# PathologyFoundation/plip

Hardware: NVIDIA H100
Metric: image-text pairs/sec (224x224, 77-tok) (higher is better)
Workload: dtype bf16

## Files before the change

### include/plip_b200.h

```cpp
#ifndef PLIP_B200_H_
#define PLIP_B200_H_

#include <stdint.h>

#ifdef __cplusplus
extern "C" {
#endif

#define PLIP_API __attribute__((visibility("default")))

#define PLIP_B200_ABI_VERSION 5

#define PLIP_IMAGE_SIZE 224
#define PLIP_EMBED_DIM 512
#define PLIP_TEXT_SEQ 77
#define PLIP_VOCAB 49408

typedef struct plip_engine plip_engine_t;

enum plip_pixel_format {
  PLIP_PIX_F32_NCHW = 0,
  PLIP_PIX_BF16_NCHW = 1,
  PLIP_PIX_U8_NHWC = 2
};

enum plip_id_dtype { PLIP_IDS_I32 = 0, PLIP_IDS_I64 = 1 };

enum plip_operand_format { PLIP_OPERAND_BF16 = 0, PLIP_OPERAND_FP16 = 1 };

PLIP_API const char* plip_last_error(void);
PLIP_API int plip_abi_version(void);
PLIP_API uint64_t plip_launch_count(void);

typedef struct plip_tensor_info {
  char name[96];
  uint64_t offset;
  uint64_t numel;
  int32_t dtype;
  int32_t rows;
  int32_t cols;
  int32_t fused;
} plip_tensor_info_t;

PLIP_API int plip_weights_num_tensors(void);
PLIP_API int plip_weights_tensor_info(int index, plip_tensor_info_t* info);
PLIP_API uint64_t plip_weights_blob_bytes(void);

PLIP_API int plip_create(const void* host_blob, uint64_t blob_bytes, float logit_scale_exp, int device,
                         int max_micro_batch, plip_engine_t** out);
PLIP_API int plip_create_ex(const void* host_blob, uint64_t blob_bytes, float logit_scale_exp, int device,
                            int max_micro_batch, int operand_format, plip_engine_t** out);
PLIP_API int plip_destroy(plip_engine_t* e);
PLIP_API uint64_t plip_workspace_bytes(int max_micro_batch);
PLIP_API float plip_logit_scale_exp(const plip_engine_t* e);
PLIP_API int plip_max_micro_batch(const plip_engine_t* e);
PLIP_API int plip_operand_format(const plip_engine_t* e);
PLIP_API int plip_set_text_pooling(plip_engine_t* e, int no_eos_argmax);
PLIP_API int plip_set_last_layer_pruning(plip_engine_t* e, int on);
PLIP_API int plip_last_layer_pruning(const plip_engine_t* e);

PLIP_API int plip_encode_images(plip_engine_t* e, const void* pixels_dev, int pixel_format, int64_t n,
                                float* out_dev, int normalize, void* stream);

PLIP_API int plip_encode_images_hw(plip_engine_t* e, const void* pixels_dev, int pixel_format, int64_t n, int height,
                                   int width, float* out_dev, int normalize, void* stream);

PLIP_API int plip_encode_windows(plip_engine_t* e, const void* region_dev, int height, int width,
                                 int64_t row_pitch_bytes, const int32_t* origins_host, int64_t n, float* out_dev,
                                 int normalize, void* stream);
PLIP_API int plip_window_background_counts(const void* region_dev, int height, int width, int64_t row_pitch_bytes,
                                           const int32_t* origins_host, int64_t n, int threshold, int32_t* counts_dev,
                                           void* stream);
PLIP_API int plip_window_mask_counts(const void* mask_dev, int height, int width, int channels,
                                     int64_t row_pitch_bytes, const int32_t* origins_host, int64_t n, int threshold,
                                     int32_t* counts_dev, void* stream);

PLIP_API int plip_encode_text(plip_engine_t* e, const void* ids_dev, int ids_dtype,
                              const void* attention_mask_dev, int64_t n, int seq_len, float* out_dev,
                              int normalize, void* stream);

PLIP_API int plip_encode_text_prefix(plip_engine_t* e, const void* ids_dev, int ids_dtype,
                                     const void* attention_mask_dev, int64_t n, int seq_len, int prefix_len,
                                     float* out_dev, int normalize, void* stream);

typedef struct plip_tower_outputs {
  float* embeds;
  float* pooled;
  float* last_hidden;
  float* hidden;
  float* attn;
  int32_t normalize;
} plip_tower_outputs_t;
PLIP_API int plip_vision_outputs(plip_engine_t* e, const void* pixels_dev, int pixel_format, int64_t n, int height,
                                 int width, const plip_tower_outputs_t* outputs, void* stream);
PLIP_API int plip_text_outputs(plip_engine_t* e, const void* ids_dev, int ids_dtype, const void* attention_mask_dev,
                               int64_t n, int seq_len, const plip_tower_outputs_t* outputs, void* stream);

PLIP_API int plip_similarity(const float* img_dev, int64_t n, const float* txt_dev, int64_t m, float scale,
                             int normalize_img, int normalize_txt, float* logits_dev, int64_t ld_logits,
                             void* stream);

PLIP_API int plip_similarity_topk(const float* query_dev, int64_t n, const float* space_dev, int64_t m,
                                  float scale, int normalize_query, int normalize_space, int k,
                                  int32_t* idx_dev, float* val_dev, void* stream);

PLIP_API int plip_l2_normalize(float* x_dev, int64_t n, int dim, void* stream);

typedef struct plip_resize_desc {
  int64_t offset;
  int32_t width, height;
  int32_t new_width, new_height;
  int32_t left, top;
} plip_resize_desc_t;
PLIP_API int plip_resize_crop_u8(const void* src_dev, uint64_t src_bytes, const plip_resize_desc_t* descs_host,
                                 int64_t n, void* tiles_dev, void* stream);
PLIP_API int plip_resize_crop_bilinear_u8(const void* src_dev, uint64_t src_bytes, const plip_resize_desc_t* descs_host,
                                          int64_t n, void* tiles_dev, void* stream);
PLIP_API int plip_resize_crop_fill_u8(const void* src_dev, uint64_t src_bytes, const plip_resize_desc_t* descs_host,
                                      int64_t n, void* tiles_dev, void* stream);

PLIP_API int plip_mask_value_sets_u8(const void* masks_dev, int64_t n, int height, int width, int channels,
                                     uint32_t* sets_dev, void* stream);

typedef struct plip_warp_desc {
  double affine[6];
  double perspective[8];
  int32_t flip;
  int32_t apply_perspective;
  int32_t fill;
  int32_t reserved;
} plip_warp_desc_t;
PLIP_API int plip_warp_tiles_u8(const void* src_dev, void* dst_dev, const plip_warp_desc_t* descs_host, int64_t n,
                                void* stream);

PLIP_API int plip_resize_region_workspace(int height, int width, int new_height, int new_width, int out_row0,
                                          int out_row1, uint64_t* bytes);
PLIP_API int plip_resize_region_u8(const void* src_dev, int64_t src_row_pitch, int src_row0, int src_rows, int height,
                                   int width, void* out_dev, int64_t out_row_pitch, int new_height, int new_width,
                                   int out_row0, int out_row1, void* workspace_dev, uint64_t workspace_bytes,
                                   void* stream);
PLIP_API int plip_resize_filter_bounds(int in_size, int out_size, int32_t* bounds_host);

typedef struct plip_sgd_problem {
  double alpha;
  double pos_weight;
  double neg_weight;
  int32_t pos_class;
  int32_t sigma_index;
} plip_sgd_problem_t;
PLIP_API int plip_sgd_shuffle_permutation(int64_t n, uint32_t seed, int32_t* sigma_host);
PLIP_API int plip_sgd_workspace_bytes(int64_t n, int n_sigma, int n_problems, uint64_t* bytes);
PLIP_API int plip_sgd_fit(const float* x_dev, int64_t n, int dim, const int32_t* class_host, int n_classes,
                          const plip_sgd_problem_t* problems_host, int n_problems, const int32_t* sigma_host,
                          int n_sigma, int max_iter, double tol, int n_iter_no_change, float* coef_dev,
                          double* intercept_dev, int32_t* n_iter_dev, int32_t* overflow_dev, void* workspace_dev,
                          uint64_t workspace_bytes, void* stream);
PLIP_API int plip_linear_decision(const float* x_dev, int64_t n, int dim, const float* coef_dev,
                                  const double* intercept_dev, int n_out, float* scores_dev, int32_t* pred_dev,
                                  void* stream);

typedef struct plip_densenet plip_densenet_t;
PLIP_API int plip_densenet_num_tensors(void);
PLIP_API int plip_densenet_tensor_info(int index, plip_tensor_info_t* info);
PLIP_API uint64_t plip_densenet_blob_bytes(void);
PLIP_API uint64_t plip_densenet_workspace_bytes(int max_micro_batch);
PLIP_API int plip_densenet_create(const void* host_blob, uint64_t blob_bytes, int device, int max_micro_batch,
                                  plip_densenet_t** out);
PLIP_API int plip_densenet_destroy(plip_densenet_t* e);
PLIP_API int plip_densenet_max_micro_batch(const plip_densenet_t* e);
PLIP_API int plip_densenet_encode(plip_densenet_t* e, const void* tiles_dev, int64_t n, float* out_dev, void* stream);

PLIP_API int plip_encode_images_host(plip_engine_t* e, const void* pixels_host, int pixel_format, int64_t n,
                                     float* out_host, int normalize);
PLIP_API int plip_encode_text_host(plip_engine_t* e, const void* ids_host, int ids_dtype,
                                   const void* attention_mask_host, int64_t n, int seq_len,
                                   float* out_host, int normalize);

typedef struct plip_kernel_time {
  char name[48];
  int32_t launches;
  float total_ms;
  double flops;
  double bytes;
} plip_kernel_time_t;
PLIP_API int plip_profile_enable(plip_engine_t* e, int on);
PLIP_API int plip_profile_read(plip_engine_t* e, plip_kernel_time_t* out, int cap, int* count);

PLIP_API int plip_dbg_set_operand_format(int operand_format);
PLIP_API int plip_dbg_gemm(const void* A_bf16, int lda, const void* W_bf16, int ldw, int M, int N, int K,
                           const float* bias, void* out, int ldo, const float* pos, int epilogue, int cluster_size,
                           int block_n, const float* colsum, const float* stats_in, int n_partials, void* xb_out,
                           float* stats_out, void* stream);
PLIP_API int plip_dbg_resize_filter(int in_size, int out_size, int xx, int32_t* k_host, int k_cap, int* xmin,
                                    int* count);
PLIP_API int plip_dbg_resize_filter_bilinear(int in_size, int out_size, int xx, int32_t* k_host, int k_cap, int* xmin,
                                             int* count);
PLIP_API int plip_dbg_text_bucket_plan(const int32_t* lens_host, int64_t n, int seq_len, int32_t* perm_host,
                                       int32_t* bucket_start_host, int32_t* bucket_prefix_host, int cap);
PLIP_API int plip_dbg_rowstats_cast(const float* x, int64_t rows, int dim, void* xb_bf16, float* stats, void* stream);
PLIP_API int plip_dbg_layernorm(const float* x, int64_t rows, int dim, int64_t in_row_stride,
                                const float* gamma, const float* beta, float* out_f32, void* out_bf16,
                                void* stream);
PLIP_API int plip_dbg_attention(const void* qkv_bf16, int64_t n_seq, int seq_len, int heads, int causal,
                                const int32_t* key_mask, void* out_bf16, void* stream);
PLIP_API int plip_dbg_attention_probs(const void* qkv_bf16, int64_t n_seq, int seq_len, int heads, int causal,
                                      const int32_t* key_mask, float* probs_dev, void* stream);
PLIP_API int plip_dbg_densenet_op(int op, const void* in_dev, int lda, int64_t n, int side, int c_in, const void* w_dev,
                                  const float* a_scale, const float* a_shift, const float* e_scale,
                                  const float* e_shift, void* out_dev, int ldo, void* stream);
PLIP_API int plip_dbg_im2col(const void* pixels, int pixel_format, int64_t n, void* out_bf16, void* stream);
PLIP_API int plip_dbg_pos_interp(const float* pos_dev, int grid_h, int grid_w, float* out_dev, void* stream);
PLIP_API int plip_dbg_hidden_states_hw(plip_engine_t* e, const void* pixels_dev, int pixel_format, int64_t n,
                                       int height, int width, int num_layers, float* hidden_dev, void* stream);
PLIP_API int plip_dbg_hidden_states(plip_engine_t* e, int tower, const void* input_dev, int input_format,
                                    const void* attention_mask_dev, int64_t n, int num_layers,
                                    float* hidden_dev, void* stream);

#ifdef __cplusplus
}
#endif
#endif
```

### plip_b200/_lib.py

```python
from __future__ import annotations

import ctypes as C
from pathlib import Path

_PKG = Path(__file__).resolve().parent
LIB_PATH = _PKG / "libplip_b200.so"

_vp = C.c_void_p
_i = C.c_int
_i64 = C.c_int64
_u64 = C.c_uint64
_f = C.c_float
_fp = C.c_void_p


class TensorInfo(C.Structure):

    _fields_ = [
        ("name", C.c_char * 96),
        ("offset", C.c_uint64),
        ("numel", C.c_uint64),
        ("dtype", C.c_int32),
        ("rows", C.c_int32),
        ("cols", C.c_int32),
        ("fused", C.c_int32),
    ]


class KernelTime(C.Structure):

    _fields_ = [("name", C.c_char * 48), ("launches", C.c_int32), ("total_ms", C.c_float), ("flops", C.c_double),
                ("bytes", C.c_double)]


class ResizeDesc(C.Structure):

    _fields_ = [
        ("offset", C.c_int64),
        ("width", C.c_int32),
        ("height", C.c_int32),
        ("new_width", C.c_int32),
        ("new_height", C.c_int32),
        ("left", C.c_int32),
        ("top", C.c_int32),
    ]


class WarpDesc(C.Structure):

    _fields_ = [("affine", C.c_double * 6), ("perspective", C.c_double * 8), ("flip", C.c_int32),
                ("apply_perspective", C.c_int32), ("fill", C.c_int32), ("reserved", C.c_int32)]


class SgdProblem(C.Structure):

    _fields_ = [("alpha", C.c_double), ("pos_weight", C.c_double), ("neg_weight", C.c_double), ("pos_class", C.c_int32),
                ("sigma_index", C.c_int32)]


class TowerOutputs(C.Structure):

    _fields_ = [("embeds", C.c_void_p), ("pooled", C.c_void_p), ("last_hidden", C.c_void_p), ("hidden", C.c_void_p),
                ("attn", C.c_void_p), ("normalize", C.c_int32)]


SIGNATURES = {
    "plip_last_error": (C.c_char_p, []),
    "plip_abi_version": (_i, []),
    "plip_launch_count": (_u64, []),
    "plip_weights_num_tensors": (_i, []),
    "plip_weights_tensor_info": (_i, [_i, C.POINTER(TensorInfo)]),
    "plip_weights_blob_bytes": (_u64, []),
    "plip_create": (_i, [_vp, _u64, _f, _i, _i, C.POINTER(_vp)]),
    "plip_create_ex": (_i, [_vp, _u64, _f, _i, _i, _i, C.POINTER(_vp)]),
    "plip_operand_format": (_i, [_vp]),
    "plip_set_text_pooling": (_i, [_vp, _i]),
    "plip_set_last_layer_pruning": (_i, [_vp, _i]),
    "plip_last_layer_pruning": (_i, [_vp]),
    "plip_dbg_set_operand_format": (_i, [_i]),
    "plip_destroy": (_i, [_vp]),
    "plip_workspace_bytes": (_u64, [_i]),
    "plip_logit_scale_exp": (_f, [_vp]),
    "plip_max_micro_batch": (_i, [_vp]),
    "plip_encode_images": (_i, [_vp, _vp, _i, _i64, _fp, _i, _vp]),
    "plip_encode_images_hw": (_i, [_vp, _vp, _i, _i64, _i, _i, _fp, _i, _vp]),
    "plip_encode_windows": (_i, [_vp, _vp, _i, _i, _i64, _vp, _i64, _fp, _i, _vp]),
    "plip_window_background_counts": (_i, [_vp, _i, _i, _i64, _vp, _i64, _i, _vp, _vp]),
    "plip_encode_text": (_i, [_vp, _vp, _i, _vp, _i64, _i, _fp, _i, _vp]),
    "plip_encode_text_prefix": (_i, [_vp, _vp, _i, _vp, _i64, _i, _i, _fp, _i, _vp]),
    "plip_vision_outputs": (_i, [_vp, _vp, _i, _i64, _i, _i, C.POINTER(TowerOutputs), _vp]),
    "plip_text_outputs": (_i, [_vp, _vp, _i, _vp, _i64, _i, C.POINTER(TowerOutputs), _vp]),
    "plip_similarity": (_i, [_fp, _i64, _fp, _i64, _f, _i, _i, _fp, _i64, _vp]),
    "plip_similarity_topk": (_i, [_fp, _i64, _fp, _i64, _f, _i, _i, _i, _vp, _fp, _vp]),
    "plip_l2_normalize": (_i, [_fp, _i64, _i, _vp]),
    "plip_window_mask_counts": (_i, [_vp, _i, _i, _i, _i64, _vp, _i64, _i, _vp, _vp]),
    "plip_resize_crop_u8": (_i, [_vp, _u64, _vp, _i64, _vp, _vp]),
    "plip_resize_crop_bilinear_u8": (_i, [_vp, _u64, _vp, _i64, _vp, _vp]),
    "plip_resize_crop_fill_u8": (_i, [_vp, _u64, _vp, _i64, _vp, _vp]),
    "plip_mask_value_sets_u8": (_i, [_vp, _i64, _i, _i, _i, _vp, _vp]),
    "plip_warp_tiles_u8": (_i, [_vp, _vp, _vp, _i64, _vp]),
    "plip_resize_region_workspace": (_i, [_i, _i, _i, _i, _i, _i, C.POINTER(_u64)]),
    "plip_resize_region_u8": (_i, [_vp, _i64, _i, _i, _i, _i, _vp, _i64, _i, _i, _i, _i, _vp, _u64, _vp]),
    "plip_resize_filter_bounds": (_i, [_i, _i, _vp]),
    "plip_sgd_shuffle_permutation": (_i, [_i64, C.c_uint32, _vp]),
    "plip_sgd_workspace_bytes": (_i, [_i64, _i, _i, C.POINTER(_u64)]),
    "plip_sgd_fit": (_i, [_fp, _i64, _i, _vp, _i, _vp, _i, _vp, _i, _i, C.c_double, _i, _fp, _vp, _vp, _vp, _vp, _u64,
                          _vp]),
    "plip_linear_decision": (_i, [_fp, _i64, _i, _fp, _vp, _i, _fp, _vp, _vp]),
    "plip_densenet_num_tensors": (_i, []),
    "plip_densenet_tensor_info": (_i, [_i, C.POINTER(TensorInfo)]),
    "plip_densenet_blob_bytes": (_u64, []),
    "plip_densenet_workspace_bytes": (_u64, [_i]),
    "plip_densenet_create": (_i, [_vp, _u64, _i, _i, C.POINTER(_vp)]),
    "plip_densenet_destroy": (_i, [_vp]),
    "plip_densenet_max_micro_batch": (_i, [_vp]),
    "plip_densenet_encode": (_i, [_vp, _vp, _i64, _fp, _vp]),
    "plip_encode_images_host": (_i, [_vp, _vp, _i, _i64, _fp, _i]),
    "plip_encode_text_host": (_i, [_vp, _vp, _i, _vp, _i64, _i, _fp, _i]),
    "plip_profile_enable": (_i, [_vp, _i]),
    "plip_profile_read": (_i, [_vp, C.POINTER(KernelTime), _i, C.POINTER(_i)]),
    "plip_dbg_gemm": (_i, [_vp, _i, _vp, _i, _i, _i, _i, _fp, _vp, _i, _fp, _i, _i, _i, _fp, _fp, _i, _vp, _fp, _vp]),
    "plip_dbg_resize_filter": (_i, [_i, _i, _i, _vp, _i, C.POINTER(_i), C.POINTER(_i)]),
    "plip_dbg_resize_filter_bilinear": (_i, [_i, _i, _i, _vp, _i, C.POINTER(_i), C.POINTER(_i)]),
    "plip_dbg_text_bucket_plan": (_i, [_vp, _i64, _i, _vp, _vp, _vp, _i]),
    "plip_dbg_rowstats_cast": (_i, [_fp, _i64, _i, _vp, _fp, _vp]),
    "plip_dbg_layernorm": (_i, [_fp, _i64, _i, _i64, _fp, _fp, _fp, _vp, _vp]),
    "plip_dbg_attention": (_i, [_vp, _i64, _i, _i, _i, _vp, _vp, _vp]),
    "plip_dbg_attention_probs": (_i, [_vp, _i64, _i, _i, _i, _vp, _fp, _vp]),
    "plip_dbg_densenet_op": (_i, [_i, _vp, _i, _i64, _i, _i, _vp, _fp, _fp, _fp, _fp, _vp, _i, _vp]),
    "plip_dbg_im2col": (_i, [_vp, _i, _i64, _vp, _vp]),
    "plip_dbg_hidden_states": (_i, [_vp, _i, _vp, _i, _vp, _i64, _i, _fp, _vp]),
    "plip_dbg_pos_interp": (_i, [_fp, _i, _i, _fp, _vp]),
    "plip_dbg_hidden_states_hw": (_i, [_vp, _vp, _i, _i64, _i, _i, _i, _fp, _vp]),
}

_LIB = None


def lib(strict: bool = True) -> C.CDLL:
    global _LIB
    if _LIB is not None:
        return _LIB
    if not LIB_PATH.exists():
        raise RuntimeError(
            f"{LIB_PATH} is missing: build it with `python -m plip_b200.build` "
            "(plip_b200 has no CPU fallback; the sm_90a CUDA library is the product)."
        )
    dll = C.CDLL(str(LIB_PATH))
    missing = []
    for name, (res, args) in SIGNATURES.items():
        try:
            fn = getattr(dll, name)
        except AttributeError:
            missing.append(name)
            continue
        fn.restype = res
        fn.argtypes = args
    if missing and strict:
        raise RuntimeError(f"{LIB_PATH} does not export: {missing}")
    _LIB = dll
    return dll


def last_error() -> str:
    msg = lib(strict=False).plip_last_error()
    return msg.decode("utf-8", "replace") if msg else ""


def check(rc: int, what: str) -> None:
    if rc != 0:
        raise RuntimeError(f"{what} failed (rc={rc}): {last_error()}")
```

### plip_b200/csrc/engine.cu

```cuda
#include "kernels.cuh"

#include <stdlib.h>
#include <string.h>

#include <array>
#include <map>
#include <string>
#include <tuple>
#include <vector>

namespace plip {
const char* get_last_error();

namespace {

struct Spec {
  std::string name;
  int dtype;
  int rows, cols, fused;
  uint64_t offset, numel;
};

void add(std::vector<Spec>& v, const std::string& name, int dtype, int rows, int cols, int fused = 0) {
  Spec s;
  s.name = name; s.dtype = dtype; s.rows = rows; s.cols = cols; s.fused = fused;
  s.numel = (uint64_t)rows * cols;
  s.offset = 0;
  v.push_back(s);
}

void add_tower(std::vector<Spec>& v, const std::string& pfx, int D, int FF) {
  for (int l = 0; l < kLayers; ++l) {
    const std::string p = pfx + ".encoder.layers." + std::to_string(l);
    add(v, p + ".self_attn.q_proj.weight", 1, 3 * D, D, 3);
    add(v, p + ".self_attn.q_proj.bias", 0, 3 * D, 1, 3);
    add(v, p + ".self_attn.q_proj.colsum", 0, 3 * D, 1, 3);
    add(v, p + ".self_attn.out_proj.weight", 1, D, D);
    add(v, p + ".self_attn.out_proj.bias", 0, D, 1);
    add(v, p + ".mlp.fc1.weight", 1, FF, D, 2);
    add(v, p + ".mlp.fc1.bias", 0, FF, 1, 2);
    add(v, p + ".mlp.fc1.colsum", 0, FF, 1, 2);
    add(v, p + ".mlp.fc2.weight", 1, D, FF);
    add(v, p + ".mlp.fc2.bias", 0, D, 1);
  }
}

std::vector<Spec> build_specs() {
  std::vector<Spec> v;
  add(v, "vision_model.embeddings.patch_embedding.weight", 1, kVisDim, kPatchK);
  add(v, "vision_model.embeddings.class_embedding", 0, kVisDim, 1);
  add(v, "vision_model.embeddings.position_embedding.weight", 0, kVisSeq, kVisDim);
  add(v, "vision_model.pre_layrnorm.weight", 0, kVisDim, 1);
  add(v, "vision_model.pre_layrnorm.bias", 0, kVisDim, 1);
  add_tower(v, "vision_model", kVisDim, kVisFF);
  add(v, "vision_model.post_layernorm.weight", 0, kVisDim, 1);
  add(v, "vision_model.post_layernorm.bias", 0, kVisDim, 1);
  add(v, "visual_projection.weight", 1, kProj, kVisDim);
  add(v, "text_model.embeddings.token_embedding.weight", 0, kVocab, kTxtDim);
  add(v, "text_model.embeddings.position_embedding.weight", 0, kTxtSeq, kTxtDim);
  add_tower(v, "text_model", kTxtDim, kTxtFF);
  add(v, "text_model.final_layer_norm.weight", 0, kTxtDim, 1);
  add(v, "text_model.final_layer_norm.bias", 0, kTxtDim, 1);
  add(v, "text_projection.weight", 1, kProj, kTxtDim);
  uint64_t off = 0;
  for (auto& s : v) {
    s.offset = off;
    off += s.numel * (s.dtype == 1 ? 2 : 4);
    off = (off + 255) & ~255ull;
  }
  return v;
}

const std::vector<Spec>& specs() {
  static const std::vector<Spec> v = build_specs();
  return v;
}

uint64_t blob_bytes() {
  const auto& v = specs();
  const Spec& s = v.back();
  return (s.offset + s.numel * (s.dtype == 1 ? 2 : 4) + 255) & ~255ull;
}

struct LayerW {
  const float *bqkv, *sqkv, *bo, *b1, *s1, *b2;
  const __nv_bfloat16 *wqkv, *wo, *w1, *w2;
};

constexpr int kEosId = 49407;

enum ProfKind { PK_QKV = 0, PK_ATTN, PK_OUT, PK_FC1, PK_FC2, PK_PATCH, PK_IM2COL, PK_LN, PK_ROWSTATS, PK_EMBED, PK_PROJ,
                PK_MISC, PK_ATTN_LONG, PK_ATTN_PROBS, PK_COUNT };
const char* const kProfNames[PK_COUNT] = {"gemm[ln1+qkv]", "attention", "gemm[out_proj+resid]", "gemm[ln2+fc1+gelu]",
                                          "gemm[fc2+resid]", "gemm[patch_embed]", "im2col", "layernorm",
                                          "rowstats_cast", "text_embed", "gemm[projection]", "misc", "attention[long]",
                                          "attention[probs]"};

size_t pixel_bytes(int fmt, int height = kImage, int width = kImage) {
  const size_t px = (size_t)3 * height * width;
  return fmt == PLIP_PIX_F32_NCHW ? px * 4 : (fmt == PLIP_PIX_BF16_NCHW ? px * 2 : px);
}

struct VisGeom {
  int H = kImage, W = kImage, gh = kGrid, gw = kGrid, S = kVisSeq;
};

VisGeom vis_geom(int height, int width) {
  VisGeom g;
  g.H = height; g.W = width; g.gh = height / kPatch; g.gw = width / kPatch; g.S = g.gh * g.gw + 1;
  return g;
}

struct VisInput {
  const void* pixels;
  int fmt;
  WindowSrc win;
};

VisInput tiles(const void* pixels, int fmt) { return VisInput{pixels, fmt, WindowSrc{nullptr, 0, nullptr}}; }

int64_t images_per_pass(int max_mb, int S) {
  const int64_t n = (int64_t)kVisSeq * max_mb / S;
  return n < max_mb ? n : max_mb;
}

struct GraphKey {
  int tower;
  int n;
  int format;
  int normalize, seq_len, prefix_len, has_mask, pool_argmax, prune;
  auto fields() const {
    return std::tie(tower, n, format, normalize, seq_len, prefix_len, has_mask, pool_argmax, prune);
  }
  bool operator<(const GraphKey& o) const { return fields() < o.fields(); }
};

struct Graph {
  cudaGraphExec_t exec = nullptr;
  unsigned long long kernels = 0;
};

}
}

using namespace plip;

struct plip_engine {
  int device = 0;
  int max_mb = 0;
  int text_pool_argmax = 0;
  int prune_last = 0;
  int f16 = 0;
  float logit_scale_exp = 1.f;
  uint8_t* d_blob = nullptr;
  const __nv_bfloat16 *v_patch_w = nullptr, *v_proj = nullptr;
  const float *v_cls = nullptr, *v_pos = nullptr, *v_pre_g = nullptr, *v_pre_b = nullptr, *v_post_g = nullptr,
              *v_post_b = nullptr;
  LayerW vis[kLayers], txt[kLayers];
  const float *t_tok = nullptr, *t_pos = nullptr, *t_fin_g = nullptr, *t_fin_b = nullptr;
  const __nv_bfloat16* t_proj = nullptr;
  float* X = nullptr;
  __nv_bfloat16* Xn = nullptr;
  __nv_bfloat16* AO = nullptr;
  float2* stats = nullptr;
  __nv_bfloat16* QKV = nullptr;
  __nv_bfloat16* H = nullptr;
  __nv_bfloat16* pooled = nullptr;
  int32_t* row_idx = nullptr;
  int32_t* kmask = nullptr;
  cudaEvent_t ev_last = nullptr;
  cudaStream_t s_compute = nullptr, s_copy = nullptr;
  cudaEvent_t ev_copied[2] = {nullptr, nullptr}, ev_done[2] = {nullptr, nullptr};
  void* d_in[2] = {nullptr, nullptr};
  size_t d_in_bytes = 0;
  void* h_stage[2] = {nullptr, nullptr};
  size_t h_stage_bytes = 0;
  float* d_out = nullptr;
  size_t d_out_bytes = 0;
  void* d_aux = nullptr;
  size_t d_aux_bytes = 0;
  int32_t* d_win = nullptr;
  size_t d_win_bytes = 0;
  int graph_max_n = 128;
  cudaStream_t s_cap = nullptr;
  void* g_in[2] = {nullptr, nullptr};
  size_t g_in_bytes[2] = {0, 0};
  float* g_out = nullptr;
  std::map<GraphKey, Graph> graphs;
  bool prof_on = false;
  int prof_tower = 0;
  std::vector<cudaEvent_t> prof_ev;
  struct ProfRec { int kind; int tower; double flops, bytes; };
  std::vector<ProfRec> prof_rec;
};

namespace {

struct ProfScope {
  plip_engine* e;
  cudaStream_t st;
  bool on;
  ProfScope(plip_engine* e_, cudaStream_t st_, int kind, double flops, double bytes) : e(e_), st(st_), on(e_->prof_on) {
    if (!on) return;
    if (e->prof_rec.size() >= 8192) { on = false; return; }
    cudaEvent_t a = nullptr, b = nullptr;
    if (cudaEventCreate(&a) != cudaSuccess || cudaEventCreate(&b) != cudaSuccess) { on = false; return; }
    e->prof_ev.push_back(a);
    e->prof_ev.push_back(b);
    e->prof_rec.push_back({kind, e->prof_tower, flops, bytes});
    cudaEventRecord(a, st);
  }
  ~ProfScope() {
    if (on) cudaEventRecord(e->prof_ev.back(), st);
  }
};

template <typename T>
const T* wptr(const plip_engine* e, const Spec& s) {
  return reinterpret_cast<const T*>(e->d_blob + s.offset);
}

int bind_weights(plip_engine* e) {
  const auto& v = specs();
  size_t i = 0;
  auto nextf = [&]() { return wptr<float>(e, v[i++]); };
  auto nextb = [&]() { return wptr<__nv_bfloat16>(e, v[i++]); };
  auto tower = [&](LayerW* L) {
    for (int l = 0; l < kLayers; ++l) {
      L[l].wqkv = nextb(); L[l].bqkv = nextf(); L[l].sqkv = nextf();
      L[l].wo = nextb(); L[l].bo = nextf();
      L[l].w1 = nextb(); L[l].b1 = nextf(); L[l].s1 = nextf();
      L[l].w2 = nextb(); L[l].b2 = nextf();
    }
  };
  e->v_patch_w = nextb();
  e->v_cls = nextf();
  e->v_pos = nextf();
  e->v_pre_g = nextf(); e->v_pre_b = nextf();
  tower(e->vis);
  e->v_post_g = nextf(); e->v_post_b = nextf();
  e->v_proj = nextb();
  e->t_tok = nextf();
  e->t_pos = nextf();
  tower(e->txt);
  e->t_fin_g = nextf(); e->t_fin_b = nextf();
  e->t_proj = nextb();
  PLIP_REQUIRE(i == v.size(), "internal: weight table mismatch (%zu vs %zu)", i, v.size());
  return 0;
}

struct WsLayout {
  size_t x, xn, ao, stats, qkv, h, pooled, rowidx, kmask, total;
};

WsLayout ws_layout(int mb) {
  const size_t rv = (size_t)mb * kVisSeq, rt = (size_t)mb * kTxtSeq;
  auto mx = [](size_t a, size_t b) { return a > b ? a : b; };
  auto al = [](size_t a) { return (a + 1023) & ~(size_t)1023; };
  WsLayout w;
  size_t off = 0;
  w.x = off; off += al(mx(rv * kVisDim, rt * kTxtDim) * 4);
  w.xn = off; off += al(mx(rv * kVisDim, rt * kTxtDim) * 2);
  w.ao = off; off += al(mx(rv * kVisDim, rt * kTxtDim) * 2);
  w.stats = off; off += al(mx(rv, rt) * kStatSlots * sizeof(float2));
  w.qkv = off; off += al(mx(rv * 3 * kVisDim, rt * 3 * kTxtDim) * 2);
  w.h = off; off += al(mx(mx(rv * kVisFF, rt * kTxtFF), (size_t)mb * kPatches * kPatchK) * 2);
  w.pooled = off; off += al((size_t)mb * kVisDim * 2);
  w.rowidx = off; off += al((size_t)mb * 4);
  w.kmask = off; off += al(rt * 4);
  w.total = off;
  return w;
}

int gemm(plip_engine* e, int kind, GemmArgs g, cudaStream_t st) {
  g.f16 = e->f16;
  const double M = g.M, N = g.N, K = g.K;
  const double out_elem = g.epi == EPI_BIAS_RESID_F32 ? 8 : (g.epi == EPI_F32 || g.epi == EPI_PATCH_F32 ? 4 : 2);
  ProfScope ps(e, st, kind, 2 * M * N * K, M * K * 2 + N * K * 2 + M * N * out_elem + (g.xb_out ? M * N * 2 : 0));
  return launch_gemm(g, st);
}

int layer_tail(plip_engine* e, const LayerW& w, int rows, int D, int FF, const __nv_bfloat16* ao, float* x, bool last,
               int& np, cudaStream_t st) {
  GemmArgs g;
  g.A = ao; g.lda = D; g.W = w.wo; g.ldw = D; g.M = rows; g.N = D; g.K = D;
  g.bias = w.bo; g.out = x; g.ldo = D; g.epi = EPI_BIAS_RESID_F32;
  g.xb_out = e->Xn; g.stats_out = e->stats; g.n_tiles_used = &np;
  if (int rc = gemm(e, PK_OUT, g, st)) return rc;
  g = GemmArgs();
  g.A = e->Xn; g.lda = D; g.W = w.w1; g.ldw = D; g.M = rows; g.N = FF; g.K = D;
  g.bias = w.b1; g.colsum = w.s1; g.stats_in = e->stats; g.n_partials = np;
  g.out = e->H; g.ldo = FF; g.epi = EPI_LN_BIAS_GELU_BF16;
  if (int rc = gemm(e, PK_FC1, g, st)) return rc;
  g = GemmArgs();
  g.A = e->H; g.lda = FF; g.W = w.w2; g.ldw = FF; g.M = rows; g.N = D; g.K = FF;
  g.bias = w.b2; g.out = x; g.ldo = D; g.epi = EPI_BIAS_RESID_F32;
  if (!last) { g.xb_out = e->Xn; g.stats_out = e->stats; g.n_tiles_used = &np; }
  return gemm(e, PK_FC2, g, st);
}

struct PassOut {
  float *embeds = nullptr, *pooled = nullptr, *last_hidden = nullptr;
  float* hidden = nullptr;
  int64_t hidden_stride = 0;
  float* attn = nullptr;
  int64_t attn_stride = 0;
  int normalize = 0;
};

PassOut pass_out(const plip_tower_outputs_t& o, int64_t n, int64_t i0, int S, int D, int heads) {
  PassOut p;
  const int64_t tok = (int64_t)S * D, pp = (int64_t)heads * S * S;
  if (o.embeds) p.embeds = o.embeds + i0 * kProj;
  if (o.pooled) p.pooled = o.pooled + i0 * D;
  if (o.last_hidden) p.last_hidden = o.last_hidden + i0 * tok;
  if (o.hidden) { p.hidden = o.hidden + i0 * tok; p.hidden_stride = n * tok; }
  if (o.attn) { p.attn = o.attn + i0 * pp; p.attn_stride = n * pp; }
  p.normalize = o.normalize;
  return p;
}

PassOut embeds_only(float* out, int normalize) {
  PassOut p;
  p.embeds = out;
  p.normalize = normalize;
  return p;
}

int run_layers(plip_engine* e, const LayerW* L, int64_t n_seq, int S, int D, int FF, int heads, bool causal,
               const int32_t* kmask, int num_layers, cudaStream_t st, bool prune = false,
               const int32_t* pool_idx = nullptr, const PassOut& out = PassOut(), const float** pooled_x = nullptr) {
  const int64_t M = n_seq * S;
  PLIP_REQUIRE(M <= 0x7fffffff / 4, "micro-batch too large");
  PLIP_REQUIRE(!prune || (pooled_x && !out.hidden && !out.attn), "internal: per-layer outputs of a pruned pass");
  const size_t x_bytes = (size_t)M * D * 4;
  if (out.hidden) PLIP_CUDA_CHECK(cudaMemcpyAsync(out.hidden, e->X, x_bytes, cudaMemcpyDeviceToDevice, st));
  if (num_layers <= 0) return 0;
  {
    ProfScope ps(e, st, PK_ROWSTATS, 0, (double)M * D * 6 + (double)M * 8);
    if (int rc = launch_rowstats_cast(e->X, M, D, e->Xn, e->stats, e->f16, st)) return rc;
  }
  const double b_att = (double)M * 3 * D * 2 + (double)M * D * 2;
  const double f_att = 4.0 * (double)n_seq * heads * S * S * kHeadDim;
  int np = 1;
  for (int l = 0; l < num_layers; ++l) {
    const LayerW& w = L[l];
    const bool last = l + 1 == num_layers;
    GemmArgs g;
    g.A = e->Xn; g.lda = D; g.W = w.wqkv; g.ldw = D; g.M = (int)M; g.N = 3 * D; g.K = D;
    g.bias = w.bqkv; g.colsum = w.sqkv; g.stats_in = e->stats; g.n_partials = np;
    g.out = e->QKV; g.ldo = 3 * D; g.epi = EPI_LN_BIAS_BF16;
    if (int rc = gemm(e, PK_QKV, g, st)) return rc;
    {
      ProfScope ps(e, st, S > 128 ? PK_ATTN_LONG : PK_ATTN, f_att, b_att);
      if (int rc = launch_attention(e->QKV, n_seq, S, heads, causal, kmask, e->AO, e->f16, st)) return rc;
    }
    if (out.attn) {
      ProfScope ps(e, st, PK_ATTN_PROBS, 0.5 * f_att, (double)M * 2 * D * 2 + (double)n_seq * heads * S * S * 4);
      if (int rc = launch_attention_probs(e->QKV, n_seq, S, heads, causal, kmask, out.attn + l * out.attn_stride,
                                          e->f16, st)) return rc;
    }
    if (!(prune && last)) {
      if (int rc = layer_tail(e, w, (int)M, D, FF, e->AO, e->X, last, np, st)) return rc;
      if (out.hidden)
        PLIP_CUDA_CHECK(cudaMemcpyAsync(out.hidden + (l + 1) * out.hidden_stride, e->X, x_bytes,
                                        cudaMemcpyDeviceToDevice, st));
      continue;
    }
    __nv_bfloat16* ao_p = e->QKV;
    float* x_p = reinterpret_cast<float*>(reinterpret_cast<uint8_t*>(e->QKV) + (((size_t)n_seq * D * 2 + 1023) & ~(size_t)1023));
    {
      ProfScope ps(e, st, PK_MISC, 0, (double)n_seq * D * 12);
      if (int rc = launch_gather_rows(e->AO, e->X, pool_idx, S, n_seq, D, ao_p, x_p, st)) return rc;
    }
    if (int rc = layer_tail(e, w, (int)n_seq, D, FF, ao_p, x_p, true, np, st)) return rc;
    *pooled_x = x_p;
  }
  return 0;
}

int vision_trunk(plip_engine* e, const VisInput& in, int64_t mb, const VisGeom& geo, int num_layers,
                 cudaStream_t st, bool prune = false, const PassOut& out = PassOut(),
                 const float** pooled_x = nullptr) {
  e->prof_tower = 0;
  const double dmb = (double)mb;
  const int patches = geo.gh * geo.gw;
  const float* pos = e->v_pos;
  if (geo.gh != kGrid || geo.gw != kGrid) {
    float* table = reinterpret_cast<float*>(e->QKV);
    ProfScope ps(e, st, PK_MISC, 0, (double)kVisSeq * kVisDim * 4 + (double)geo.S * kVisDim * 4);
    if (int rc = launch_pos_interp(e->v_pos, geo.gh, geo.gw, table, st)) return rc;
    pos = table;
  }
  {
    ProfScope ps(e, st, PK_IM2COL, 0, dmb * (double)pixel_bytes(in.fmt, geo.H, geo.W) + dmb * patches * kPatchK * 2);
    const int rc = in.win.region ? launch_window_im2col(in.win, mb, e->H, e->f16, st)
                                 : launch_im2col(in.pixels, in.fmt, mb, geo.H, geo.W, e->H, e->f16, st);
    if (rc) return rc;
  }
  GemmArgs g;
  g.A = e->H; g.lda = kPatchK; g.W = e->v_patch_w; g.ldw = kPatchK;
  g.M = (int)(mb * patches); g.N = kVisDim; g.K = kPatchK;
  g.out = e->X; g.ldo = kVisDim; g.pos = pos; g.patches = patches; g.seq = geo.S; g.epi = EPI_PATCH_F32;
  if (int rc = gemm(e, PK_PATCH, g, st)) return rc;
  {
    ProfScope ps(e, st, PK_MISC, 0, dmb * kVisDim * 4);
    if (int rc = launch_cls_rows(e->v_cls, pos, mb, geo.S, e->X, st)) return rc;
  }
  const int64_t M = mb * geo.S;
  {
    ProfScope ps(e, st, PK_LN, 0, (double)M * kVisDim * 8);
    if (int rc = launch_layernorm(e->X, nullptr, kVisDim, M, kVisDim, e->v_pre_g, e->v_pre_b, e->X, nullptr, e->f16, st)) return rc;
  }
  return run_layers(e, e->vis, mb, geo.S, kVisDim, kVisFF, kVisHeads, false, nullptr, num_layers, st, prune, nullptr,
                    out, pooled_x);
}

int pooled_head(plip_engine* e, const float* pooled_x, const int32_t* pool_idx, int64_t mb, int S, int D,
                const float* gamma, const float* beta, const __nv_bfloat16* proj, float* out, int normalize,
                cudaStream_t st, float* pooled_f32) {
  {
    ProfScope ps(e, st, PK_LN, 0, (double)mb * D * (pooled_f32 ? 10 : 6));
    const bool compact = pooled_x != nullptr;
    if (int rc = launch_layernorm(compact ? pooled_x : e->X, compact ? nullptr : pool_idx,
                                  compact || pool_idx ? (int64_t)D : (int64_t)S * D, mb, D, gamma, beta, pooled_f32,
                                  e->pooled, e->f16, st)) return rc;
  }
  if (!out) return 0;
  GemmArgs g;
  g.A = e->pooled; g.lda = D; g.W = proj; g.ldw = D;
  g.M = (int)mb; g.N = kProj; g.K = D; g.out = out; g.ldo = kProj; g.epi = EPI_F32;
  if (int rc = gemm(e, PK_PROJ, g, st)) return rc;
  if (normalize) {
    ProfScope ps(e, st, PK_MISC, 0, (double)mb * kProj * 8);
    return launch_l2_normalize(out, mb, kProj, st);
  }
  return 0;
}

int vision_pass(plip_engine* e, const VisInput& in, int64_t mb, const VisGeom& geo, const PassOut& out, bool prune,
                cudaStream_t st) {
  const float* pooled_x = nullptr;
  if (int rc = vision_trunk(e, in, mb, geo, kLayers, st, prune, out, &pooled_x)) return rc;
  if (out.last_hidden)
    PLIP_CUDA_CHECK(cudaMemcpyAsync(out.last_hidden, e->X, (size_t)mb * geo.S * kVisDim * 4, cudaMemcpyDeviceToDevice,
                                    st));
  if (!out.embeds && !out.pooled) return 0;
  return pooled_head(e, pooled_x, nullptr, mb, geo.S, kVisDim, e->v_post_g, e->v_post_b, e->v_proj, out.embeds,
                     out.normalize, st, out.pooled);
}

int text_trunk(plip_engine* e, const void* ids, int ids_dtype, const void* mask, int64_t mb, int S, int stride,
               int num_layers, cudaStream_t st, bool prune = false, const PassOut& out = PassOut(),
               const float** pooled_x = nullptr) {
  e->prof_tower = 1;
  {
    ProfScope ps(e, st, PK_EMBED, 0, (double)mb * S * kTxtDim * 8);
    if (int rc = launch_text_embed(ids, ids_dtype, mb, S, stride, e->t_tok, e->t_pos, e->X, e->row_idx, kEosId, e->text_pool_argmax, st)) return rc;
  }
  const int32_t* km = nullptr;
  if (mask) {
    ProfScope ps(e, st, PK_MISC, 0, (double)mb * S * 12);
    if (int rc = launch_mask_to_i32(mask, ids_dtype, mb * S, S, stride, e->kmask, st)) return rc;
    km = e->kmask;
  }
  return run_layers(e, e->txt, mb, S, kTxtDim, kTxtFF, kTxtHeads, true, km, num_layers, st, prune, e->row_idx, out,
                    pooled_x);
}

int text_pass(plip_engine* e, const void* ids, int ids_dtype, const void* mask, int64_t mb, int S, int stride,
              const PassOut& out, bool prune, cudaStream_t st) {
  const float* pooled_x = nullptr;
  if (int rc = text_trunk(e, ids, ids_dtype, mask, mb, S, stride, kLayers, st, prune, out, &pooled_x)) return rc;
  if (out.last_hidden) {
    ProfScope ps(e, st, PK_LN, 0, (double)mb * S * kTxtDim * 8);
    if (int rc = launch_layernorm(e->X, nullptr, kTxtDim, mb * S, kTxtDim, e->t_fin_g, e->t_fin_b, out.last_hidden,
                                  nullptr, e->f16, st)) return rc;
  }
  if (!out.embeds && !out.pooled) return 0;
  return pooled_head(e, pooled_x, e->row_idx, mb, S, kTxtDim, e->t_fin_g, e->t_fin_b, e->t_proj, out.embeds,
                     out.normalize, st, out.pooled);
}

int ensure_host_path(plip_engine* e) {
  if (e->s_compute) return 0;
  PLIP_CUDA_CHECK(cudaStreamCreateWithFlags(&e->s_compute, cudaStreamNonBlocking));
  PLIP_CUDA_CHECK(cudaStreamCreateWithFlags(&e->s_copy, cudaStreamNonBlocking));
  for (int i = 0; i < 2; ++i) {
    PLIP_CUDA_CHECK(cudaEventCreateWithFlags(&e->ev_copied[i], cudaEventDisableTiming));
    PLIP_CUDA_CHECK(cudaEventCreateWithFlags(&e->ev_done[i], cudaEventDisableTiming));
  }
  return 0;
}

int grow_dev(void** p, size_t* have, size_t want) {
  if (*have >= want) return 0;
  if (*p) PLIP_CUDA_CHECK(cudaFree(*p));
  *p = nullptr; *have = 0;
  PLIP_CUDA_CHECK(cudaMalloc(p, want));
  *have = want;
  return 0;
}

constexpr long long kMinBucketRows = 8192, kBucketOverheadRows = 2048;
constexpr int kMaxTextBuckets = 8;

int plan_text_buckets(const int32_t* lens, int64_t n, int seq_len, int32_t* perm, int32_t* start, int32_t* prefix,
                      int cap) {
  std::vector<int64_t> upto(seq_len + 1, 0);
  for (int64_t i = 0; i < n; ++i) {
    const int L = lens[i] < 1 ? 1 : (lens[i] > seq_len ? seq_len : lens[i]);
    ++upto[L];
  }
  std::vector<int64_t> first(seq_len + 2, 0);
  for (int L = 1; L <= seq_len; ++L) first[L + 1] = first[L] + upto[L];
  if (perm) {
    std::vector<int64_t> cur(first.begin(), first.end());
    for (int64_t i = 0; i < n; ++i) {
      const int L = lens[i] < 1 ? 1 : (lens[i] > seq_len ? seq_len : lens[i]);
      perm[cur[L]++] = (int32_t)i;
    }
  }
  std::vector<int> ends;
  for (int L = 1; L <= seq_len; ++L)
    if (upto[L]) ends.push_back(L);
  for (int L = 1; L <= seq_len; ++L) upto[L] += upto[L - 1];
  const int m = (int)ends.size();
  const int kb = cap < kMaxTextBuckets ? cap : kMaxTextBuckets;
  const long long INF = 1LL << 62;
  std::vector<std::vector<long long>> f(kb, std::vector<long long>(m, INF));
  std::vector<std::vector<int>> from(kb, std::vector<int>(m, -1));
  auto cost = [&](int jlo, int jhi) {
    const long long cnt = upto[ends[jhi]] - (jlo ? upto[ends[jlo - 1]] : 0);
    const long long rows = cnt * ends[jhi];
    return (rows < kMinBucketRows ? kMinBucketRows : rows) + kBucketOverheadRows;
  };
  for (int j = 0; j < m; ++j) f[0][j] = cost(0, j);
  for (int b = 1; b < kb; ++b)
    for (int j = b; j < m; ++j)
      for (int i = b - 1; i < j; ++i)
        if (f[b - 1][i] < INF) {
          const long long c = f[b - 1][i] + cost(i + 1, j);
          if (c < f[b][j]) f[b][j] = c, from[b][j] = i;
        }
  int best_b = 0;
  for (int b = 1; b < kb; ++b)
    if (m > b && f[b][m - 1] < f[best_b][m - 1]) best_b = b;
  const int nb = best_b + 1;
  int j = m - 1;
  for (int b = best_b; b >= 0; --b) {
    prefix[b] = ends[j];
    const int i = b ? from[b][j] : -1;
    start[b] = (int32_t)(i >= 0 ? upto[ends[i]] : 0);
    j = i;
  }
  start[nb] = (int32_t)n;
  return nb;
}

bool is_pinned(const void* p) {
  cudaPointerAttributes a;
  if (cudaPointerGetAttributes(&a, p) != cudaSuccess) {
    cudaGetLastError();
    return false;
  }
  return a.type == cudaMemoryTypeHost;
}

}

namespace {

int count_kernel_nodes(cudaGraph_t g, unsigned long long* kernels) {
  size_t n = 0;
  PLIP_CUDA_CHECK(cudaGraphGetNodes(g, nullptr, &n));
  std::vector<cudaGraphNode_t> nodes(n);
  PLIP_CUDA_CHECK(cudaGraphGetNodes(g, nodes.data(), &n));
  *kernels = 0;
  for (cudaGraphNode_t node : nodes) {
    cudaGraphNodeType type;
    PLIP_CUDA_CHECK(cudaGraphNodeGetType(node, &type));
    *kernels += type == cudaGraphNodeTypeKernel;
  }
  return 0;
}

template <typename F>
int capture_graph(plip_engine* e, F&& body, Graph* out) {
  if (!e->s_cap) PLIP_CUDA_CHECK(cudaStreamCreateWithFlags(&e->s_cap, cudaStreamNonBlocking));
  PLIP_CUDA_CHECK(cudaStreamBeginCapture(e->s_cap, cudaStreamCaptureModeThreadLocal));
  int rc = body(e->s_cap);
  cudaGraph_t g = nullptr;
  const cudaError_t ce = cudaStreamEndCapture(e->s_cap, &g);
  if (g) {
    const int rc_count = count_kernel_nodes(g, &out->kernels);
    if (rc == 0) rc = rc_count;
    g_launch_count.fetch_sub(out->kernels, std::memory_order_relaxed);
  }
  if (rc != 0) {
    if (g) cudaGraphDestroy(g);
    return rc;
  }
  PLIP_CUDA_CHECK(ce);
  const cudaError_t ci = cudaGraphInstantiate(&out->exec, g, 0);
  cudaGraphDestroy(g);
  PLIP_CUDA_CHECK(ci);
  return 0;
}

int check_pixels(const char* fn, const plip_engine* e, const void* in, const void* out, int fmt, int64_t n,
                 int height, int width) {
  PLIP_REQUIRE(in && out, "%s: null argument", fn);
  PLIP_REQUIRE(n > 0, "%s: n must be positive (got %lld)", fn, (long long)n);
  PLIP_REQUIRE(fmt >= 0 && fmt <= 2, "%s: unknown pixel format %d", fn, fmt);
  PLIP_REQUIRE(height >= kPatch && width >= kPatch && height / kPatch <= kMaxGrid && width / kPatch <= kMaxGrid,
               "%s: image size %dx%d out of range (32 <= height, width and at most %d patches of 32 per side)", fn,
               height, width, kMaxGrid);
  PLIP_REQUIRE(e != nullptr, "%s: null engine", fn);
  const int S = (height / kPatch) * (width / kPatch) + 1;
  PLIP_REQUIRE(S <= (int64_t)kVisSeq * e->max_mb,
               "%s: a %dx%d image has %d tokens, more than the %lld token rows of the workspace "
               "(%d x max_micro_batch %d); create the engine with max_micro_batch >= %d",
               fn, height, width, S, (long long)kVisSeq * e->max_mb, kVisSeq, e->max_mb, (S + kVisSeq - 1) / kVisSeq);
  return 0;
}

int check_ids(const char* fn, const plip_engine* e, const void* ids, const void* out, int ids_dtype, int64_t n,
              int seq_len, int prefix_len) {
  PLIP_REQUIRE(ids && out, "%s: null argument", fn);
  PLIP_REQUIRE(n > 0, "%s: n must be positive (got %lld)", fn, (long long)n);
  PLIP_REQUIRE(seq_len >= 1 && seq_len <= kTxtSeq,
               "Sequence length must be less than max_position_embeddings (got `sequence length`: %d and "
               "max_position_embeddings: %d)", seq_len, kTxtSeq);
  PLIP_REQUIRE(prefix_len >= 1 && prefix_len <= seq_len, "%s: prefix_len %d out of [1,%d]", fn, prefix_len, seq_len);
  PLIP_REQUIRE(ids_dtype == PLIP_IDS_I32 || ids_dtype == PLIP_IDS_I64, "%s: unknown ids dtype %d", fn, ids_dtype);
  PLIP_REQUIRE(e != nullptr, "%s: null engine", fn);
  return 0;
}

int check_outputs(const char* fn, const plip_tower_outputs_t* o) {
  PLIP_REQUIRE(o != nullptr, "%s: null outputs", fn);
  PLIP_REQUIRE(o->embeds || o->pooled || o->last_hidden || o->hidden || o->attn, "%s: no output requested", fn);
  return 0;
}

int check_windows(const char* fn, const void* region, int height, int width, int64_t row_pitch,
                  const int32_t* origins, int64_t n, const void* out, int channels = 3) {
  PLIP_REQUIRE(region && origins && out, "%s: null argument", fn);
  PLIP_REQUIRE(n > 0, "%s: n must be positive (got %lld)", fn, (long long)n);
  PLIP_REQUIRE(height >= kImage && width >= kImage, "%s: region %dx%d is smaller than one %dx%d window", fn, height,
               width, kImage, kImage);
  PLIP_REQUIRE(row_pitch >= (int64_t)channels * width, "%s: row pitch %lld bytes < %d * width = %lld", fn,
               (long long)row_pitch, channels, (long long)channels * width);
  for (int64_t i = 0; i < n; ++i) {
    const int r = origins[2 * i], c = origins[2 * i + 1];
    PLIP_REQUIRE(r >= 0 && c >= 0 && r <= height - kImage && c <= width - kImage,
                 "%s: window %lld at (%d, %d) is outside the %dx%d region (rows 0..%d, columns 0..%d)", fn,
                 (long long)i, r, c, height, width, height - kImage, width - kImage);
  }
  return 0;
}

template <typename F>
int micro_batches(plip_engine* e, int64_t n, int64_t per_pass, cudaStream_t st, F&& pass) {
  PLIP_CUDA_CHECK(cudaStreamWaitEvent(st, e->ev_last, 0));
  for (int64_t i = 0; i < n; i += per_pass)
    if (int rc = pass(i, n - i < per_pass ? n - i : per_pass)) return rc;
  PLIP_CUDA_CHECK(cudaEventRecord(e->ev_last, st));
  return 0;
}

bool graph_eligible(const plip_engine* e, int64_t n) {
  return e->graph_max_n > 0 && n <= e->graph_max_n && n <= e->max_mb && !e->prof_on;
}

constexpr size_t kMaxGraphs = 96;
void trim_graphs(plip_engine* e) {
  if (e->graphs.size() < kMaxGraphs) return;
  cudaDeviceSynchronize();
  for (auto& kv : e->graphs) cudaGraphExecDestroy(kv.second.exec);
  e->graphs.clear();
}

struct Staged {
  const void* src;
  size_t bytes;
};

template <typename F>
int graph_call(plip_engine* e, const GraphKey& key, std::array<Staged, 2> in, float* out, cudaStream_t st,
               F&& forward) {
  PLIP_CUDA_CHECK(cudaStreamWaitEvent(st, e->ev_last, 0));
  auto it = e->graphs.find(key);
  if (it == e->graphs.end()) {
    const size_t stage_bytes[2] = {(size_t)e->graph_max_n * pixel_bytes(PLIP_PIX_F32_NCHW),
                                   (size_t)e->graph_max_n * kTxtSeq * 8};
    for (int i = 0; i < 2; ++i)
      if (in[i].src)
        if (int rc = grow_dev(&e->g_in[i], &e->g_in_bytes[i], stage_bytes[i])) return rc;
    if (!e->g_out) PLIP_CUDA_CHECK(cudaMalloc(&e->g_out, (size_t)e->graph_max_n * kProj * 4));
    if (int rc = forward(st, in[0].src, in[1].src, out)) return rc;
    Graph graph;
    if (int rc = capture_graph(e, [&](cudaStream_t cs) {
          return forward(cs, in[0].src ? e->g_in[0] : nullptr, in[1].src ? e->g_in[1] : nullptr, e->g_out);
        }, &graph)) return rc;
    trim_graphs(e);
    e->graphs.emplace(key, graph);
  } else {
    for (int i = 0; i < 2; ++i)
      if (in[i].src) PLIP_CUDA_CHECK(cudaMemcpyAsync(e->g_in[i], in[i].src, in[i].bytes, cudaMemcpyDeviceToDevice, st));
    PLIP_CUDA_CHECK(cudaGraphLaunch(it->second.exec, st));
    PLIP_CUDA_CHECK(cudaMemcpyAsync(out, e->g_out, (size_t)key.n * kProj * 4, cudaMemcpyDeviceToDevice, st));
    g_launch_count.fetch_add(it->second.kernels, std::memory_order_relaxed);
  }
  PLIP_CUDA_CHECK(cudaEventRecord(e->ev_last, st));
  return 0;
}

int dbg_hidden_states(const char* fn, plip_engine* e, int tower, const void* in, int fmt, const void* mask, int64_t n,
                      int height, int width, int num_layers, float* hidden, cudaStream_t st) {
  PLIP_REQUIRE(tower == 0 || tower == 1, "%s: tower %d out of range (0 vision, 1 text)", fn, tower);
  PLIP_REQUIRE(num_layers >= 0 && num_layers <= kLayers, "%s: num_layers %d out of range", fn, num_layers);
  if (int rc = tower == 0 ? check_pixels(fn, e, in, hidden, fmt, n, height, width)
                          : check_ids(fn, e, in, hidden, fmt, n, kTxtSeq, kTxtSeq)) return rc;
  const VisGeom geo = vis_geom(height, width);
  const int S = tower == 0 ? geo.S : kTxtSeq, D = tower == 0 ? kVisDim : kTxtDim;
  const int64_t per_pass = tower == 0 ? images_per_pass(e->max_mb, S) : e->max_mb;
  PLIP_REQUIRE(n <= per_pass, "%s: n=%lld sequences of %d tokens exceed one pass (%lld)", fn, (long long)n, S,
               (long long)per_pass);
  return micro_batches(e, n, n, st, [&](int64_t, int64_t) {
    if (int rc = tower == 0 ? vision_trunk(e, tiles(in, fmt), n, geo, num_layers, st)
                            : text_trunk(e, in, fmt, mask, n, kTxtSeq, kTxtSeq, num_layers, st)) return rc;
    PLIP_CUDA_CHECK(cudaMemcpyAsync(hidden, e->X, (size_t)n * S * D * 4, cudaMemcpyDeviceToDevice, st));
    return 0;
  });
}

}

extern "C" {

PLIP_API const char* plip_last_error(void) { return plip::get_last_error(); }
PLIP_API int plip_abi_version(void) { return PLIP_B200_ABI_VERSION; }
PLIP_API uint64_t plip_launch_count(void) { return plip::g_launch_count.load(std::memory_order_relaxed); }

PLIP_API int plip_weights_num_tensors(void) { return (int)specs().size(); }

PLIP_API int plip_weights_tensor_info(int index, plip_tensor_info_t* info) {
  const auto& v = specs();
  PLIP_REQUIRE(info != nullptr && index >= 0 && index < (int)v.size(), "tensor_info: index %d out of range", index);
  memset(info, 0, sizeof(*info));
  strncpy(info->name, v[index].name.c_str(), sizeof(info->name) - 1);
  info->offset = v[index].offset;
  info->numel = v[index].numel;
  info->dtype = v[index].dtype;
  info->rows = v[index].rows;
  info->cols = v[index].cols;
  info->fused = v[index].fused;
  return 0;
}

PLIP_API uint64_t plip_weights_blob_bytes(void) { return blob_bytes(); }

PLIP_API uint64_t plip_workspace_bytes(int max_micro_batch) {
  return max_micro_batch > 0 ? ws_layout(max_micro_batch).total : 0;
}

PLIP_API int plip_create(const void* host_blob, uint64_t nbytes, float logit_scale_exp, int device,
                         int max_micro_batch, plip_engine_t** out) {
  return plip_create_ex(host_blob, nbytes, logit_scale_exp, device, max_micro_batch, PLIP_OPERAND_BF16, out);
}

PLIP_API int plip_create_ex(const void* host_blob, uint64_t nbytes, float logit_scale_exp, int device,
                            int max_micro_batch, int operand_format, plip_engine_t** out) {
  PLIP_REQUIRE(out != nullptr && host_blob != nullptr, "plip_create: null argument");
  PLIP_REQUIRE(operand_format == PLIP_OPERAND_BF16 || operand_format == PLIP_OPERAND_FP16,
               "plip_create: unknown operand format %d", operand_format);
  PLIP_REQUIRE(nbytes == blob_bytes(), "plip_create: blob is %llu bytes, expected %llu",
               (unsigned long long)nbytes, (unsigned long long)blob_bytes());
  PLIP_REQUIRE(max_micro_batch >= 1 && max_micro_batch <= 8192, "plip_create: max_micro_batch %d out of [1,8192]",
               max_micro_batch);
  int ndev = 0;
  PLIP_CUDA_CHECK(cudaGetDeviceCount(&ndev));
  PLIP_REQUIRE(device >= 0 && device < ndev, "plip_create: device %d not present (%d devices)", device, ndev);
  PLIP_CUDA_CHECK(cudaSetDevice(device));
  cudaDeviceProp prop;
  PLIP_CUDA_CHECK(cudaGetDeviceProperties(&prop, device));
  PLIP_REQUIRE(prop.major == 9 && prop.minor == 0, "plip_create: device %d is sm_%d%d; this library is built for sm_90a only",
               device, prop.major, prop.minor);
  plip_engine* e = new plip_engine();
  e->device = device;
  e->max_mb = max_micro_batch;
  e->f16 = operand_format == PLIP_OPERAND_FP16 ? 1 : 0;
  if (const char* gm = getenv("PLIP_GRAPH_MAX")) e->graph_max_n = atoi(gm) < 0 ? 0 : (atoi(gm) > 1024 ? 1024 : atoi(gm));
  e->logit_scale_exp = logit_scale_exp;
  const WsLayout w = ws_layout(max_micro_batch);
  uint8_t* ws = nullptr;
  cudaError_t ce = cudaEventCreateWithFlags(&e->ev_last, cudaEventDisableTiming);
  if (ce == cudaSuccess) ce = cudaMalloc(&e->d_blob, nbytes);
  if (ce == cudaSuccess) ce = cudaMalloc(&ws, w.total);
  e->X = reinterpret_cast<float*>(ws);
  if (ce != cudaSuccess) {
    set_last_error("plip_create: allocating %llu (weights) + %llu (workspace) bytes on device %d failed: %s",
                   (unsigned long long)nbytes, (unsigned long long)w.total, device, cudaGetErrorString(ce));
    cudaGetLastError();
    plip_destroy(e);
    return -1;
  }
  e->Xn = reinterpret_cast<__nv_bfloat16*>(ws + w.xn);
  e->AO = reinterpret_cast<__nv_bfloat16*>(ws + w.ao);
  e->stats = reinterpret_cast<float2*>(ws + w.stats);
  e->QKV = reinterpret_cast<__nv_bfloat16*>(ws + w.qkv);
  e->H = reinterpret_cast<__nv_bfloat16*>(ws + w.h);
  e->pooled = reinterpret_cast<__nv_bfloat16*>(ws + w.pooled);
  e->row_idx = reinterpret_cast<int32_t*>(ws + w.rowidx);
  e->kmask = reinterpret_cast<int32_t*>(ws + w.kmask);
  ce = cudaMemcpy(e->d_blob, host_blob, nbytes, cudaMemcpyHostToDevice);
  if (ce != cudaSuccess) {
    set_last_error("plip_create: weight upload failed: %s", cudaGetErrorString(ce));
    plip_destroy(e);
    return -1;
  }
  if (bind_weights(e) != 0) {
    plip_destroy(e);
    return -1;
  }
  *out = e;
  return 0;
}

PLIP_API int plip_destroy(plip_engine_t* e) {
  if (!e) return 0;
  cudaSetDevice(e->device);
  cudaDeviceSynchronize();
  if (e->d_blob) cudaFree(e->d_blob);
  if (e->X) cudaFree(e->X);
  for (int i = 0; i < 2; ++i) {
    if (e->d_in[i]) cudaFree(e->d_in[i]);
    if (e->h_stage[i]) cudaFreeHost(e->h_stage[i]);
    if (e->ev_copied[i]) cudaEventDestroy(e->ev_copied[i]);
    if (e->ev_done[i]) cudaEventDestroy(e->ev_done[i]);
  }
  if (e->d_out) cudaFree(e->d_out);
  if (e->d_aux) cudaFree(e->d_aux);
  if (e->d_win) cudaFree(e->d_win);
  if (e->ev_last) cudaEventDestroy(e->ev_last);
  for (auto& kv : e->graphs) cudaGraphExecDestroy(kv.second.exec);
  for (void* p : e->g_in)
    if (p) cudaFree(p);
  if (e->g_out) cudaFree(e->g_out);
  if (e->s_cap) cudaStreamDestroy(e->s_cap);
  for (cudaEvent_t ev : e->prof_ev) cudaEventDestroy(ev);
  if (e->s_compute) cudaStreamDestroy(e->s_compute);
  if (e->s_copy) cudaStreamDestroy(e->s_copy);
  delete e;
  return 0;
}

PLIP_API int plip_profile_enable(plip_engine_t* e, int on) {
  PLIP_REQUIRE(e != nullptr, "plip_profile_enable: null engine");
  for (cudaEvent_t ev : e->prof_ev) cudaEventDestroy(ev);
  e->prof_ev.clear();
  e->prof_rec.clear();
  e->prof_on = on != 0;
  return 0;
}

PLIP_API int plip_profile_read(plip_engine_t* e, plip_kernel_time_t* out, int cap, int* count) {
  PLIP_REQUIRE(e && out && count && cap > 0, "plip_profile_read: bad argument");
  plip_kernel_time_t agg[2 * PK_COUNT];
  memset(agg, 0, sizeof(agg));
  for (size_t i = 0; i < e->prof_rec.size(); ++i) {
    PLIP_CUDA_CHECK(cudaEventSynchronize(e->prof_ev[2 * i + 1]));
    float ms = 0.f;
    PLIP_CUDA_CHECK(cudaEventElapsedTime(&ms, e->prof_ev[2 * i], e->prof_ev[2 * i + 1]));
    plip_kernel_time_t& a = agg[e->prof_rec[i].tower * PK_COUNT + e->prof_rec[i].kind];
    a.launches += 1;
    a.total_ms += ms;
    a.flops += e->prof_rec[i].flops;
    a.bytes += e->prof_rec[i].bytes;
  }
  int n = 0;
  for (int t = 0; t < 2; ++t)
    for (int k = 0; k < PK_COUNT; ++k) {
      const plip_kernel_time_t& a = agg[t * PK_COUNT + k];
      if (a.launches == 0) continue;
      if (n < cap) {
        out[n] = a;
        snprintf(out[n].name, sizeof(out[n].name), "%s/%s", t == 0 ? "vision" : "text", kProfNames[k]);
      }
      ++n;
    }
  *count = n;
  return 0;
}

PLIP_API float plip_logit_scale_exp(const plip_engine_t* e) { return e ? e->logit_scale_exp : 0.f; }
PLIP_API int plip_max_micro_batch(const plip_engine_t* e) { return e ? e->max_mb : 0; }
PLIP_API int plip_operand_format(const plip_engine_t* e) { return e ? e->f16 : -1; }
PLIP_API int plip_set_text_pooling(plip_engine_t* e, int no_eos_argmax) {
  PLIP_REQUIRE(e != nullptr, "plip_set_text_pooling: null engine");
  e->text_pool_argmax = no_eos_argmax != 0;
  return 0;
}

PLIP_API int plip_set_last_layer_pruning(plip_engine_t* e, int on) {
  PLIP_REQUIRE(e != nullptr, "plip_set_last_layer_pruning: null engine");
  e->prune_last = on != 0;
  return 0;
}
PLIP_API int plip_last_layer_pruning(const plip_engine_t* e) { return e ? e->prune_last : -1; }

PLIP_API int plip_encode_images(plip_engine_t* e, const void* pixels_dev, int pixel_format, int64_t n,
                                float* out_dev, int normalize, void* stream) {
  return plip_encode_images_hw(e, pixels_dev, pixel_format, n, kImage, kImage, out_dev, normalize, stream);
}

PLIP_API int plip_encode_images_hw(plip_engine_t* e, const void* pixels_dev, int pixel_format, int64_t n, int height,
                                   int width, float* out_dev, int normalize, void* stream) {
  if (int rc = check_pixels("plip_encode_images_hw", e, pixels_dev, out_dev, pixel_format, n, height, width)) return rc;
  const VisGeom geo = vis_geom(height, width);
  const size_t pb = pixel_bytes(pixel_format, height, width);
  const bool prune = e->prune_last != 0;
  cudaStream_t st = static_cast<cudaStream_t>(stream);
  if (height == kImage && width == kImage && graph_eligible(e, n)) {
    const GraphKey key{0, (int)n, pixel_format, normalize ? 1 : 0, 0, 0, 0, 0, e->prune_last};
    return graph_call(e, key, {{{pixels_dev, (size_t)n * pb}, {nullptr, 0}}}, out_dev, st,
                      [&](cudaStream_t s, const void* pixels, const void*, float* out) {
                        return vision_pass(e, tiles(pixels, pixel_format), n, geo, embeds_only(out, normalize), prune,
                                           s);
                      });
  }
  return micro_batches(e, n, images_per_pass(e->max_mb, geo.S), st, [&](int64_t i, int64_t mb) {
    return vision_pass(e, tiles(static_cast<const uint8_t*>(pixels_dev) + i * pb, pixel_format), mb, geo,
                       embeds_only(out_dev + i * kProj, normalize), prune, st);
  });
}

PLIP_API int plip_encode_windows(plip_engine_t* e, const void* region_dev, int height, int width,
                                 int64_t row_pitch_bytes, const int32_t* origins_host, int64_t n, float* out_dev,
                                 int normalize, void* stream) {
  if (int rc = check_windows("plip_encode_windows", region_dev, height, width, row_pitch_bytes, origins_host, n,
                             out_dev)) return rc;
  PLIP_REQUIRE(e != nullptr, "plip_encode_windows: null engine");
  cudaStream_t st = static_cast<cudaStream_t>(stream);
  PLIP_CUDA_CHECK(cudaStreamWaitEvent(st, e->ev_last, 0));
  if (int rc = grow_dev(reinterpret_cast<void**>(&e->d_win), &e->d_win_bytes, (size_t)n * 2 * sizeof(int32_t)))
    return rc;
  PLIP_CUDA_CHECK(cudaMemcpyAsync(e->d_win, origins_host, (size_t)n * 2 * sizeof(int32_t), cudaMemcpyHostToDevice, st));
  const bool prune = e->prune_last != 0;
  const uint8_t* region = static_cast<const uint8_t*>(region_dev);
  return micro_batches(e, n, images_per_pass(e->max_mb, kVisSeq), st, [&](int64_t i, int64_t mb) {
    const VisInput in{nullptr, PLIP_PIX_U8_NHWC, WindowSrc{region, row_pitch_bytes, e->d_win + 2 * i}};
    return vision_pass(e, in, mb, VisGeom(), embeds_only(out_dev + i * kProj, normalize), prune, st);
  });
}

PLIP_API int plip_window_background_counts(const void* region_dev, int height, int width, int64_t row_pitch_bytes,
                                           const int32_t* origins_host, int64_t n, int threshold, int32_t* counts_dev,
                                           void* stream) {
  if (int rc = check_windows("plip_window_background_counts", region_dev, height, width, row_pitch_bytes,
                             origins_host, n, counts_dev)) return rc;
  return launch_window_background(static_cast<const uint8_t*>(region_dev), row_pitch_bytes, origins_host, n, threshold,
                                  counts_dev, static_cast<cudaStream_t>(stream));
}

PLIP_API int plip_window_mask_counts(const void* mask_dev, int height, int width, int channels,
                                     int64_t row_pitch_bytes, const int32_t* origins_host, int64_t n, int threshold,
                                     int32_t* counts_dev, void* stream) {
  PLIP_REQUIRE(channels == 1 || channels == 3, "plip_window_mask_counts: channels must be 1 or 3 (got %d)", channels);
  if (int rc = check_windows("plip_window_mask_counts", mask_dev, height, width, row_pitch_bytes, origins_host, n,
                             counts_dev, channels)) return rc;
  return launch_window_mask(static_cast<const uint8_t*>(mask_dev), row_pitch_bytes, channels, origins_host, n,
                            threshold, counts_dev, static_cast<cudaStream_t>(stream));
}

PLIP_API int plip_encode_text(plip_engine_t* e, const void* ids_dev, int ids_dtype, const void* attention_mask_dev,
                              int64_t n, int seq_len, float* out_dev, int normalize, void* stream) {
  return plip_encode_text_prefix(e, ids_dev, ids_dtype, attention_mask_dev, n, seq_len, seq_len, out_dev, normalize,
                                 stream);
}

PLIP_API int plip_encode_text_prefix(plip_engine_t* e, const void* ids_dev, int ids_dtype,
                                     const void* attention_mask_dev, int64_t n, int seq_len, int prefix_len,
                                     float* out_dev, int normalize, void* stream) {
  if (int rc = check_ids("plip_encode_text", e, ids_dev, out_dev, ids_dtype, n, seq_len, prefix_len)) return rc;
  const size_t row = (size_t)seq_len * (ids_dtype == PLIP_IDS_I64 ? 8 : 4);
  const bool prune = e->prune_last != 0;
  cudaStream_t st = static_cast<cudaStream_t>(stream);
  if (graph_eligible(e, n)) {
    const GraphKey key{1, (int)n, ids_dtype, normalize ? 1 : 0, seq_len, prefix_len, attention_mask_dev ? 1 : 0,
                       e->text_pool_argmax, e->prune_last};
    return graph_call(e, key, {{{ids_dev, n * row}, {attention_mask_dev, n * row}}}, out_dev, st,
                      [&](cudaStream_t s, const void* ids, const void* mask, float* out) {
                        return text_pass(e, ids, ids_dtype, mask, n, prefix_len, seq_len, embeds_only(out, normalize),
                                         prune, s);
                      });
  }
  return micro_batches(e, n, e->max_mb, st, [&](int64_t i, int64_t mb) {
    const uint8_t* mask = attention_mask_dev ? static_cast<const uint8_t*>(attention_mask_dev) + i * row : nullptr;
    return text_pass(e, static_cast<const uint8_t*>(ids_dev) + i * row, ids_dtype, mask, mb, prefix_len, seq_len,
                     embeds_only(out_dev + i * kProj, normalize), prune, st);
  });
}

PLIP_API int plip_vision_outputs(plip_engine_t* e, const void* pixels_dev, int pixel_format, int64_t n, int height,
                                 int width, const plip_tower_outputs_t* outputs, void* stream) {
  if (int rc = check_outputs("plip_vision_outputs", outputs)) return rc;
  if (int rc = check_pixels("plip_vision_outputs", e, pixels_dev, outputs, pixel_format, n, height, width)) return rc;
  const VisGeom geo = vis_geom(height, width);
  const size_t pb = pixel_bytes(pixel_format, height, width);
  cudaStream_t st = static_cast<cudaStream_t>(stream);
  return micro_batches(e, n, images_per_pass(e->max_mb, geo.S), st, [&](int64_t i, int64_t mb) {
    return vision_pass(e, tiles(static_cast<const uint8_t*>(pixels_dev) + i * pb, pixel_format), mb, geo,
                       pass_out(*outputs, n, i, geo.S, kVisDim, kVisHeads), false, st);
  });
}

PLIP_API int plip_text_outputs(plip_engine_t* e, const void* ids_dev, int ids_dtype, const void* attention_mask_dev,
                               int64_t n, int seq_len, const plip_tower_outputs_t* outputs, void* stream) {
  if (int rc = check_outputs("plip_text_outputs", outputs)) return rc;
  if (int rc = check_ids("plip_text_outputs", e, ids_dev, outputs, ids_dtype, n, seq_len, seq_len)) return rc;
  const size_t row = (size_t)seq_len * (ids_dtype == PLIP_IDS_I64 ? 8 : 4);
  cudaStream_t st = static_cast<cudaStream_t>(stream);
  return micro_batches(e, n, e->max_mb, st, [&](int64_t i, int64_t mb) {
    const uint8_t* mask = attention_mask_dev ? static_cast<const uint8_t*>(attention_mask_dev) + i * row : nullptr;
    return text_pass(e, static_cast<const uint8_t*>(ids_dev) + i * row, ids_dtype, mask, mb, seq_len, seq_len,
                     pass_out(*outputs, n, i, seq_len, kTxtDim, kTxtHeads), false, st);
  });
}

PLIP_API int plip_similarity(const float* img_dev, int64_t n, const float* txt_dev, int64_t m, float scale,
                             int normalize_img, int normalize_txt, float* logits_dev, int64_t ld_logits,
                             void* stream) {
  PLIP_REQUIRE(img_dev && txt_dev && logits_dev, "plip_similarity: null argument");
  cudaStream_t st = static_cast<cudaStream_t>(stream);
  const int64_t chunk = 65535LL * 64;
  for (int64_t i = 0; i < n; i += chunk) {
    const int64_t rows = n - i < chunk ? n - i : chunk;
    if (int rc = launch_similarity(img_dev + i * kProj, rows, txt_dev, m, scale, normalize_img != 0,
                                   normalize_txt != 0, logits_dev + i * ld_logits, ld_logits, st)) return rc;
  }
  return 0;
}

PLIP_API int plip_similarity_topk(const float* query_dev, int64_t n, const float* space_dev, int64_t m, float scale,
                                  int normalize_query, int normalize_space, int k, int32_t* idx_dev, float* val_dev,
                                  void* stream) {
  PLIP_REQUIRE(query_dev && space_dev && idx_dev, "plip_similarity_topk: null argument");
  return launch_similarity_topk(query_dev, n, space_dev, m, scale, normalize_query != 0, normalize_space != 0, k,
                                idx_dev, val_dev, static_cast<cudaStream_t>(stream));
}

PLIP_API int plip_l2_normalize(float* x_dev, int64_t n, int dim, void* stream) {
  PLIP_REQUIRE(x_dev, "plip_l2_normalize: null argument");
  return launch_l2_normalize(x_dev, n, dim, static_cast<cudaStream_t>(stream));
}

PLIP_API int plip_resize_crop_u8(const void* src_dev, uint64_t src_bytes, const plip_resize_desc_t* descs_host,
                                 int64_t n, void* tiles_dev, void* stream) {
  PLIP_REQUIRE(src_dev && descs_host && tiles_dev, "plip_resize_crop_u8: null argument");
  PLIP_REQUIRE(n > 0, "plip_resize_crop_u8: n must be positive (got %lld)", (long long)n);
  return launch_resize_crop(static_cast<const uint8_t*>(src_dev), (size_t)src_bytes, descs_host, n,
                            static_cast<uint8_t*>(tiles_dev), static_cast<cudaStream_t>(stream));
}

PLIP_API int plip_resize_crop_bilinear_u8(const void* src_dev, uint64_t src_bytes, const plip_resize_desc_t* descs_host,
                                          int64_t n, void* tiles_dev, void* stream) {
  PLIP_REQUIRE(src_dev && descs_host && tiles_dev, "plip_resize_crop_bilinear_u8: null argument");
  PLIP_REQUIRE(n > 0, "plip_resize_crop_bilinear_u8: n must be positive (got %lld)", (long long)n);
  return launch_resize_crop(static_cast<const uint8_t*>(src_dev), (size_t)src_bytes, descs_host, n,
                            static_cast<uint8_t*>(tiles_dev), static_cast<cudaStream_t>(stream), true);
}

PLIP_API int plip_resize_crop_fill_u8(const void* src_dev, uint64_t src_bytes, const plip_resize_desc_t* descs_host,
                                      int64_t n, void* tiles_dev, void* stream) {
  PLIP_REQUIRE(src_dev && descs_host && tiles_dev, "plip_resize_crop_fill_u8: null argument");
  PLIP_REQUIRE(n > 0, "plip_resize_crop_fill_u8: n must be positive (got %lld)", (long long)n);
  return launch_resize_crop(static_cast<const uint8_t*>(src_dev), (size_t)src_bytes, descs_host, n,
                            static_cast<uint8_t*>(tiles_dev), static_cast<cudaStream_t>(stream), false, true);
}

PLIP_API int plip_mask_value_sets_u8(const void* masks_dev, int64_t n, int height, int width, int channels,
                                     uint32_t* sets_dev, void* stream) {
  return launch_mask_value_sets(static_cast<const uint8_t*>(masks_dev), n, height, width, channels, sets_dev,
                                static_cast<cudaStream_t>(stream));
}

PLIP_API int plip_warp_tiles_u8(const void* src_dev, void* dst_dev, const plip_warp_desc_t* descs_host, int64_t n,
                                void* stream) {
  return launch_warp_tiles(static_cast<const uint8_t*>(src_dev), static_cast<uint8_t*>(dst_dev), descs_host, n,
                           static_cast<cudaStream_t>(stream));
}

PLIP_API int plip_resize_region_workspace(int height, int width, int new_height, int new_width, int out_row0,
                                          int out_row1, uint64_t* bytes) {
  PLIP_REQUIRE(bytes, "plip_resize_region_workspace: null argument");
  return resize_region_workspace(height, width, new_height, new_width, out_row0, out_row1, bytes);
}

PLIP_API int plip_resize_region_u8(const void* src_dev, int64_t src_row_pitch, int src_row0, int src_rows, int height,
                                   int width, void* out_dev, int64_t out_row_pitch, int new_height, int new_width,
                                   int out_row0, int out_row1, void* workspace_dev, uint64_t workspace_bytes,
                                   void* stream) {
  PLIP_REQUIRE(src_dev && out_dev && workspace_dev, "plip_resize_region_u8: null argument");
  return launch_resize_region(static_cast<const uint8_t*>(src_dev), src_row_pitch, src_row0, src_rows, height, width,
                              static_cast<uint8_t*>(out_dev), out_row_pitch, new_height, new_width, out_row0, out_row1,
                              static_cast<uint8_t*>(workspace_dev), workspace_bytes, static_cast<cudaStream_t>(stream));
}

PLIP_API int plip_resize_filter_bounds(int in_size, int out_size, int32_t* bounds_host) {
  PLIP_REQUIRE(bounds_host, "plip_resize_filter_bounds: null argument");
  PLIP_REQUIRE(in_size >= 1 && out_size >= 1 && in_size <= 65536 && out_size <= 65536,
               "plip_resize_filter_bounds: sizes %d -> %d are outside 1..65536", in_size, out_size);
  return resize_filter_bounds(in_size, out_size, bounds_host);
}

PLIP_API int plip_sgd_shuffle_permutation(int64_t n, uint32_t seed, int32_t* sigma_host) {
  return sgd_shuffle_permutation(n, seed, sigma_host);
}

PLIP_API int plip_sgd_workspace_bytes(int64_t n, int n_sigma, int n_problems, uint64_t* bytes) {
  return sgd_workspace_bytes(n, n_sigma, n_problems, bytes);
}

PLIP_API int plip_sgd_fit(const float* x_dev, int64_t n, int dim, const int32_t* class_host, int n_classes,
                          const plip_sgd_problem_t* problems_host, int n_problems, const int32_t* sigma_host,
                          int n_sigma, int max_iter, double tol, int n_iter_no_change, float* coef_dev,
                          double* intercept_dev, int32_t* n_iter_dev, int32_t* overflow_dev, void* workspace_dev,
                          uint64_t workspace_bytes, void* stream) {
  return launch_sgd_fit(x_dev, n, dim, class_host, n_classes, problems_host, n_problems, sigma_host, n_sigma, max_iter,
                        tol, n_iter_no_change, coef_dev, intercept_dev, n_iter_dev, overflow_dev, workspace_dev,
                        workspace_bytes, static_cast<cudaStream_t>(stream));
}

PLIP_API int plip_linear_decision(const float* x_dev, int64_t n, int dim, const float* coef_dev,
                                  const double* intercept_dev, int n_out, float* scores_dev, int32_t* pred_dev,
                                  void* stream) {
  return launch_linear_decision(x_dev, n, dim, coef_dev, intercept_dev, n_out, scores_dev, pred_dev,
                                static_cast<cudaStream_t>(stream));
}

PLIP_API int plip_dbg_resize_filter(int in_size, int out_size, int xx, int32_t* k_host, int k_cap, int* xmin,
                                    int* count) {
  PLIP_REQUIRE(k_host && xmin && count && in_size > 0 && out_size > 0 && xx >= 0 && xx < out_size,
               "plip_dbg_resize_filter: bad argument");
  return resize_filter_host(in_size, out_size, xx, k_host, k_cap, xmin, count);
}

PLIP_API int plip_dbg_resize_filter_bilinear(int in_size, int out_size, int xx, int32_t* k_host, int k_cap, int* xmin,
                                             int* count) {
  PLIP_REQUIRE(k_host && xmin && count && in_size > 0 && out_size > 0 && xx >= 0 && xx < out_size,
               "plip_dbg_resize_filter_bilinear: bad argument");
  return resize_filter_bilinear_host(in_size, out_size, xx, k_host, k_cap, xmin, count);
}

PLIP_API int plip_encode_images_host(plip_engine_t* e, const void* pixels_host, int pixel_format, int64_t n,
                                     float* out_host, int normalize) {
  if (int rc = check_pixels("plip_encode_images_host", e, pixels_host, out_host, pixel_format, n, kImage, kImage))
    return rc;
  PLIP_CUDA_CHECK(cudaSetDevice(e->device));
  if (int rc = ensure_host_path(e)) return rc;
  PLIP_CUDA_CHECK(cudaStreamWaitEvent(e->s_compute, e->ev_last, 0));
  const size_t pb = pixel_bytes(pixel_format);
  const int64_t chunk = e->max_mb;
  const size_t in_bytes = (size_t)(n < chunk ? n : chunk) * pb;
  if (e->d_in_bytes < in_bytes) {
    size_t have0 = e->d_in_bytes, have1 = e->d_in_bytes;
    if (int rc = grow_dev(&e->d_in[0], &have0, in_bytes)) return rc;
    if (int rc = grow_dev(&e->d_in[1], &have1, in_bytes)) return rc;
    e->d_in_bytes = in_bytes;
  }
  if (int rc = grow_dev(reinterpret_cast<void**>(&e->d_out), &e->d_out_bytes, (size_t)n * kProj * 4)) return rc;
  const bool pinned = is_pinned(pixels_host);
  if (!pinned && e->h_stage_bytes < in_bytes) {
    for (int i = 0; i < 2; ++i) {
      if (e->h_stage[i]) cudaFreeHost(e->h_stage[i]);
      e->h_stage[i] = nullptr;
      PLIP_CUDA_CHECK(cudaMallocHost(&e->h_stage[i], in_bytes));
    }
    e->h_stage_bytes = in_bytes;
  }
  int64_t ci = 0;
  for (int64_t i = 0; i < n; i += chunk, ++ci) {
    const int b = (int)(ci & 1);
    const int64_t mb = (n - i < chunk) ? (n - i) : chunk;
    const uint8_t* src = static_cast<const uint8_t*>(pixels_host) + (size_t)i * pb;
    if (ci >= 2) PLIP_CUDA_CHECK(cudaStreamWaitEvent(e->s_copy, e->ev_done[b], 0));
    if (!pinned) {
      if (ci >= 2) PLIP_CUDA_CHECK(cudaEventSynchronize(e->ev_copied[b]));
      memcpy(e->h_stage[b], src, (size_t)mb * pb);
      src = static_cast<const uint8_t*>(e->h_stage[b]);
    }
    PLIP_CUDA_CHECK(cudaMemcpyAsync(e->d_in[b], src, (size_t)mb * pb, cudaMemcpyHostToDevice, e->s_copy));
    PLIP_CUDA_CHECK(cudaEventRecord(e->ev_copied[b], e->s_copy));
    PLIP_CUDA_CHECK(cudaStreamWaitEvent(e->s_compute, e->ev_copied[b], 0));
    if (int rc = vision_pass(e, tiles(e->d_in[b], pixel_format), mb, VisGeom(),
                             embeds_only(e->d_out + i * kProj, normalize), e->prune_last != 0, e->s_compute)) return rc;
    PLIP_CUDA_CHECK(cudaEventRecord(e->ev_done[b], e->s_compute));
  }
  PLIP_CUDA_CHECK(cudaMemcpyAsync(out_host, e->d_out, (size_t)n * kProj * 4, cudaMemcpyDeviceToHost, e->s_compute));
  PLIP_CUDA_CHECK(cudaStreamSynchronize(e->s_compute));
  return 0;
}

PLIP_API int plip_encode_text_host(plip_engine_t* e, const void* ids_host, int ids_dtype, const void* attention_mask_host,
                                   int64_t n, int seq_len, float* out_host, int normalize) {
  if (int rc = check_ids("plip_encode_text_host", e, ids_host, out_host, ids_dtype, n, seq_len, seq_len)) return rc;
  PLIP_CUDA_CHECK(cudaSetDevice(e->device));
  if (int rc = ensure_host_path(e)) return rc;
  PLIP_CUDA_CHECK(cudaStreamWaitEvent(e->s_compute, e->ev_last, 0));
  const size_t isz = ids_dtype == PLIP_IDS_I64 ? 8 : 4;
  const size_t ib = (size_t)n * seq_len * isz;
  const size_t ib_al = (ib + 255) & ~(size_t)255;
  if (int rc = grow_dev(&e->d_aux, &e->d_aux_bytes, 2 * ib_al)) return rc;
  if (int rc = grow_dev(reinterpret_cast<void**>(&e->d_out), &e->d_out_bytes, (size_t)n * kProj * 4)) return rc;
  uint8_t* d_ids = static_cast<uint8_t*>(e->d_aux);
  uint8_t* d_mask = attention_mask_host ? d_ids + ib_al : nullptr;
  PLIP_REQUIRE(n <= 0x7fffffff, "plip_encode_text_host: n too large");
  std::vector<int32_t> lens((size_t)n);
  for (int64_t b = 0; b < n; ++b) {
    int len = seq_len;
    for (int t = 0; t < seq_len; ++t) {
      const long long id = ids_dtype == PLIP_IDS_I64 ? static_cast<const long long*>(ids_host)[b * seq_len + t]
                                                     : (long long)static_cast<const int*>(ids_host)[b * seq_len + t];
      if (id == kEosId) { len = t + 1; break; }
    }
    lens[(size_t)b] = len;
  }
  std::vector<int32_t> perm((size_t)n);
  int32_t start[kMaxTextBuckets + 1], prefix[kMaxTextBuckets];
  const int nb = plan_text_buckets(lens.data(), n, seq_len, perm.data(), start, prefix, kMaxTextBuckets);
  if (nb == 1) {
    PLIP_CUDA_CHECK(cudaMemcpyAsync(d_ids, ids_host, ib, cudaMemcpyHostToDevice, e->s_compute));
    if (d_mask) PLIP_CUDA_CHECK(cudaMemcpyAsync(d_mask, attention_mask_host, ib, cudaMemcpyHostToDevice, e->s_compute));
    if (int rc = plip_encode_text_prefix(e, d_ids, ids_dtype, d_mask, n, seq_len, prefix[0], e->d_out, normalize,
                                         e->s_compute)) return rc;
    PLIP_CUDA_CHECK(cudaMemcpyAsync(out_host, e->d_out, (size_t)n * kProj * 4, cudaMemcpyDeviceToHost, e->s_compute));
    PLIP_CUDA_CHECK(cudaStreamSynchronize(e->s_compute));
    return 0;
  }
  const size_t row_bytes = (size_t)seq_len * isz;
  std::vector<uint8_t> sorted(ib);
  for (int64_t i = 0; i < n; ++i)
    memcpy(sorted.data() + (size_t)i * row_bytes, static_cast<const uint8_t*>(ids_host) + (size_t)perm[(size_t)i] * row_bytes,
           row_bytes);
  PLIP_CUDA_CHECK(cudaMemcpyAsync(d_ids, sorted.data(), ib, cudaMemcpyHostToDevice, e->s_compute));
  PLIP_CUDA_CHECK(cudaStreamSynchronize(e->s_compute));
  if (d_mask) {
    for (int64_t i = 0; i < n; ++i)
      memcpy(sorted.data() + (size_t)i * row_bytes,
             static_cast<const uint8_t*>(attention_mask_host) + (size_t)perm[(size_t)i] * row_bytes, row_bytes);
    PLIP_CUDA_CHECK(cudaMemcpyAsync(d_mask, sorted.data(), ib, cudaMemcpyHostToDevice, e->s_compute));
    PLIP_CUDA_CHECK(cudaStreamSynchronize(e->s_compute));
  }
  for (int k = 0; k < nb; ++k) {
    const int64_t r0 = start[k], cnt = start[k + 1] - start[k];
    if (cnt <= 0) continue;
    if (int rc = plip_encode_text_prefix(e, d_ids + (size_t)r0 * row_bytes, ids_dtype,
                                         d_mask ? d_mask + (size_t)r0 * row_bytes : nullptr, cnt, seq_len, prefix[k],
                                         e->d_out + r0 * kProj, normalize, e->s_compute)) return rc;
  }
  std::vector<float> tmp((size_t)n * kProj);
  PLIP_CUDA_CHECK(cudaMemcpyAsync(tmp.data(), e->d_out, (size_t)n * kProj * 4, cudaMemcpyDeviceToHost, e->s_compute));
  PLIP_CUDA_CHECK(cudaStreamSynchronize(e->s_compute));
  for (int64_t i = 0; i < n; ++i)
    memcpy(out_host + (size_t)perm[(size_t)i] * kProj, tmp.data() + (size_t)i * kProj, (size_t)kProj * 4);
  return 0;
}

PLIP_API int plip_dbg_text_bucket_plan(const int32_t* lens_host, int64_t n, int seq_len, int32_t* perm_host,
                                       int32_t* bucket_start_host, int32_t* bucket_prefix_host, int cap) {
  if (!lens_host || !bucket_start_host || !bucket_prefix_host || n <= 0 || seq_len < 1 || seq_len > kTxtSeq || cap < 1) {
    set_last_error("plip_dbg_text_bucket_plan: bad argument");
    return -2;
  }
  return plan_text_buckets(lens_host, n, seq_len, perm_host, bucket_start_host, bucket_prefix_host, cap);
}

static int g_dbg_f16 = 0;
PLIP_API int plip_dbg_set_operand_format(int operand_format) {
  PLIP_REQUIRE(operand_format == PLIP_OPERAND_BF16 || operand_format == PLIP_OPERAND_FP16,
               "plip_dbg_set_operand_format: unknown operand format %d", operand_format);
  g_dbg_f16 = operand_format == PLIP_OPERAND_FP16 ? 1 : 0;
  return 0;
}

PLIP_API int plip_dbg_gemm(const void* A_bf16, int lda, const void* W_bf16, int ldw, int M, int N, int K,
                           const float* bias, void* out, int ldo, const float* pos, int epilogue, int cluster_size,
                           int block_n, const float* colsum, const float* stats_in, int n_partials, void* xb_out,
                           float* stats_out, void* stream) {
  GemmArgs g;
  g.A = static_cast<const __nv_bfloat16*>(A_bf16); g.lda = lda;
  g.W = static_cast<const __nv_bfloat16*>(W_bf16); g.ldw = ldw;
  g.M = M; g.N = N; g.K = K;
  g.bias = bias; g.out = out; g.ldo = ldo; g.pos = pos; g.epi = epilogue;
  g.colsum = colsum; g.stats_in = reinterpret_cast<const float2*>(stats_in); g.n_partials = n_partials;
  g.xb_out = static_cast<__nv_bfloat16*>(xb_out); g.stats_out = reinterpret_cast<float2*>(stats_out);
  g.force_cg = cluster_size; g.force_bn = block_n;
  g.f16 = g_dbg_f16;
  return launch_gemm(g, static_cast<cudaStream_t>(stream));
}

PLIP_API int plip_dbg_rowstats_cast(const float* x, int64_t rows, int dim, void* xb_bf16, float* stats, void* stream) {
  return launch_rowstats_cast(x, rows, dim, static_cast<__nv_bfloat16*>(xb_bf16), reinterpret_cast<float2*>(stats),
                              g_dbg_f16, static_cast<cudaStream_t>(stream));
}

PLIP_API int plip_dbg_layernorm(const float* x, int64_t rows, int dim, int64_t in_row_stride, const float* gamma,
                                const float* beta, float* out_f32, void* out_bf16, void* stream) {
  return launch_layernorm(x, nullptr, in_row_stride, rows, dim, gamma, beta, out_f32,
                          static_cast<__nv_bfloat16*>(out_bf16), g_dbg_f16, static_cast<cudaStream_t>(stream));
}

PLIP_API int plip_dbg_attention(const void* qkv_bf16, int64_t n_seq, int seq_len, int heads, int causal,
                                const int32_t* key_mask, void* out_bf16, void* stream) {
  return launch_attention(static_cast<const __nv_bfloat16*>(qkv_bf16), n_seq, seq_len, heads, causal != 0, key_mask,
                          static_cast<__nv_bfloat16*>(out_bf16), g_dbg_f16, static_cast<cudaStream_t>(stream));
}

PLIP_API int plip_dbg_attention_probs(const void* qkv_bf16, int64_t n_seq, int seq_len, int heads, int causal,
                                      const int32_t* key_mask, float* probs_dev, void* stream) {
  return launch_attention_probs(static_cast<const __nv_bfloat16*>(qkv_bf16), n_seq, seq_len, heads, causal != 0,
                                key_mask, probs_dev, g_dbg_f16, static_cast<cudaStream_t>(stream));
}

PLIP_API int plip_dbg_im2col(const void* pixels, int pixel_format, int64_t n, void* out_bf16, void* stream) {
  return launch_im2col(pixels, pixel_format, n, kImage, kImage, static_cast<__nv_bfloat16*>(out_bf16), g_dbg_f16,
                       static_cast<cudaStream_t>(stream));
}

PLIP_API int plip_dbg_pos_interp(const float* pos_dev, int grid_h, int grid_w, float* out_dev, void* stream) {
  return launch_pos_interp(pos_dev, grid_h, grid_w, out_dev, static_cast<cudaStream_t>(stream));
}

PLIP_API int plip_dbg_hidden_states(plip_engine_t* e, int tower, const void* input_dev, int input_format,
                                    const void* attention_mask_dev, int64_t n, int num_layers, float* hidden_dev,
                                    void* stream) {
  return dbg_hidden_states("plip_dbg_hidden_states", e, tower, input_dev, input_format, attention_mask_dev, n, kImage,
                           kImage, num_layers, hidden_dev, static_cast<cudaStream_t>(stream));
}

PLIP_API int plip_dbg_hidden_states_hw(plip_engine_t* e, const void* pixels_dev, int pixel_format, int64_t n,
                                       int height, int width, int num_layers, float* hidden_dev, void* stream) {
  return dbg_hidden_states("plip_dbg_hidden_states_hw", e, 0, pixels_dev, pixel_format, nullptr, n, height, width,
                           num_layers, hidden_dev, static_cast<cudaStream_t>(stream));
}

}
```

### plip_b200/distributed.py

```python
from __future__ import annotations

from typing import Callable, Iterable, List, Optional, Sequence, Tuple, Union

import torch
import torch.distributed as dist


def world() -> Tuple[int, int]:
    if dist.is_available() and dist.is_initialized():
        return dist.get_rank(), dist.get_world_size()
    return 0, 1


def shard_counts(n: int, world_size: int) -> List[int]:
    base, rem = divmod(int(n), int(world_size))
    return [base + (1 if r < rem else 0) for r in range(world_size)]


def shard_range(n: int, rank: int, world_size: int) -> Tuple[int, int]:
    counts = shard_counts(n, world_size)
    lo = sum(counts[:rank])
    return lo, lo + counts[rank]


def all_gather_rows(local: torch.Tensor, counts: Optional[Sequence[int]] = None, group=None) -> torch.Tensor:
    rank, ws = world()
    if ws == 1:
        return local
    local = local.contiguous()
    if counts is None:
        sizes = torch.tensor([local.shape[0]], device=local.device, dtype=torch.int64)
        all_sizes = [torch.zeros_like(sizes) for _ in range(ws)]
        dist.all_gather(all_sizes, sizes, group=group)
        counts = [int(s.item()) for s in all_sizes]
    counts = list(counts)
    if local.shape[0] != counts[rank]:
        raise ValueError(f"rank {rank}: local block has {local.shape[0]} rows, expected {counts[rank]}")
    mx = max(counts)
    d = local.shape[1:]
    if local.shape[0] < mx:
        pad = torch.zeros((mx - local.shape[0], *d), device=local.device, dtype=local.dtype)
        send = torch.cat([local, pad], dim=0)
    else:
        send = local
    recv = torch.empty((ws * mx, *d), device=local.device, dtype=local.dtype)
    dist.all_gather_into_tensor(recv, send, group=group)
    if all(c == mx for c in counts):
        return recv
    return torch.cat([recv[r * mx: r * mx + counts[r]] for r in range(ws)], dim=0)


def all_gather_rows_async(local: torch.Tensor, group=None):
    rank, ws = world()
    if ws == 1:
        return local, None
    local = local.contiguous()
    recv = torch.empty((ws * local.shape[0], *local.shape[1:]), device=local.device, dtype=local.dtype)
    work = dist.all_gather_into_tensor(recv, local, group=group, async_op=True)
    return recv, work


def _encode_chunks(encode: Callable, rows: Union[torch.Tensor, Iterable[torch.Tensor]]) -> torch.Tensor:
    if torch.is_tensor(rows):
        return encode(rows)
    return torch.cat([encode(c) for c in rows], dim=0)


class ShardedCLIP:

    def __init__(self, encode_images: Callable, encode_text: Callable, similarity: Callable, logit_scale_exp: float,
                 topk: Optional[Callable] = None):
        self.encode_images = encode_images
        self.encode_text = encode_text
        self.similarity = similarity
        self.topk = topk
        self.logit_scale_exp = float(logit_scale_exp)
        self.rank, self.world_size = world()

    @classmethod
    def from_engine(cls, engine) -> "ShardedCLIP":
        return cls(lambda x: engine.encode_images(x, normalize=True),
                   lambda ids: engine.encode_text(ids, normalize=True),
                   lambda a, b, s: engine.similarity(a, b, scale=s, normalize_image=False, normalize_text=False),
                   engine.logit_scale_exp,
                   topk=lambda q, sp, k: engine.similarity_topk(q, sp, k, scale=1.0, normalize_query=False,
                                                                normalize_space=False))

    def clip_forward(self, local_pixels, local_ids):
        txt = self.encode_text(local_ids)
        txt_all, work = all_gather_rows_async(txt)
        img = _encode_chunks(self.encode_images, local_pixels)
        if work is not None:
            work.wait()
        return self.similarity(img, txt_all, self.logit_scale_exp)

    def local_slice(self, n_total: int) -> slice:
        lo, hi = shard_range(n_total, self.rank, self.world_size)
        return slice(lo, hi)

    def zero_shot(self, local_images, class_token_ids, n_total_images: int, gather_embeddings: bool = True):
        txt = self.encode_text(class_token_ids)
        img = _encode_chunks(self.encode_images, local_images)
        logits = self.similarity(img, txt, self.logit_scale_exp)
        pred = logits.argmax(dim=-1)
        all_img = None
        if gather_embeddings:
            all_img = all_gather_rows(img, shard_counts(n_total_images, self.world_size))
        return pred, logits, all_img

    def retrieval(self, local_gallery_images, local_query_ids, n_total_queries: int):
        q_local = self.encode_text(local_query_ids)
        counts = shard_counts(n_total_queries, self.world_size)
        if self.world_size > 1 and len(set(counts)) == 1:
            q_all, work = all_gather_rows_async(q_local)
            gal = _encode_chunks(self.encode_images, local_gallery_images)
            work.wait()
        else:
            gal = _encode_chunks(self.encode_images, local_gallery_images)
            q_all = all_gather_rows(q_local, counts)
        block = self.similarity(gal, q_all, self.logit_scale_exp)
        return block, gal, q_all

    def retrieval_topk(self, gal_local: torch.Tensor, q_all: torch.Tensor, k: int, n_total_gallery: int):
        if self.topk is None:
            raise RuntimeError("ShardedCLIP was built without a top-k kernel")
        idx, val = self.topk(q_all, gal_local, k)
        lo, _ = shard_range(n_total_gallery, self.rank, self.world_size)
        gidx = idx.to(torch.int64) + lo
        gidx = torch.where(idx < 0, torch.full_like(gidx, -1), gidx)
        if self.world_size == 1:
            return gidx, val
        nq = q_all.shape[0]
        cand_v = all_gather_rows(val.contiguous()).view(self.world_size, nq, k).permute(1, 0, 2).reshape(nq, -1)
        cand_i = all_gather_rows(gidx.contiguous()).view(self.world_size, nq, k).permute(1, 0, 2).reshape(nq, -1)
        cand_v = torch.where(cand_i < 0, torch.full_like(cand_v, float("-inf")), cand_v)
        order = torch.sort(cand_v, dim=1, descending=True, stable=True).indices[:, :k]
        return torch.gather(cand_i, 1, order), torch.gather(cand_v, 1, order)
```

### plip_b200/engine.py

```python
from __future__ import annotations

import ctypes as C
from typing import Dict, Mapping, Optional, Tuple, Union

import numpy as np
import torch

from ._lib import SgdProblem as _SgdProblem
from ._lib import check, lib
from .weights import operand_format, pack_state_dict

PIX_F32_NCHW, PIX_BF16_NCHW, PIX_U8_NHWC = 0, 1, 2
IDS_I32, IDS_I64 = 0, 1
EMBED_DIM = 512
IMAGE_SIZE = 224
MAX_TEXT_LEN = 77


VISION_DIM, VISION_HEADS = 768, 12
TEXT_DIM, TEXT_HEADS = 512, 8
NUM_LAYERS = 12

PATCH = 32
MAX_GRID = 32


def _check_size(h: int, w: int, interpolate_pos_encoding: bool) -> None:
    if not interpolate_pos_encoding:
        if h != IMAGE_SIZE or w != IMAGE_SIZE:
            raise ValueError(f"Input image size ({h}*{w}) doesn't match model (224*224).")
    elif not (h >= PATCH and w >= PATCH and h // PATCH <= MAX_GRID and w // PATCH <= MAX_GRID):
        raise ValueError(f"Input image size ({h}*{w}) out of range for interpolate_pos_encoding: height and width "
                         f"must be >= {PATCH} with at most {MAX_GRID} patches of {PATCH} per side (<= 1055 px)")


def _pixel_format(t: Union[torch.Tensor, np.ndarray], interpolate_pos_encoding: bool = False) -> int:
    shape, dtype = tuple(t.shape), t.dtype
    if dtype in (torch.uint8, np.dtype("uint8")):
        if len(shape) != 4 or shape[3] != 3:
            raise ValueError(f"uint8 images must be [n,224,224,3] (NHWC), got {shape}")
        _check_size(shape[1], shape[2], interpolate_pos_encoding)
        return PIX_U8_NHWC
    if len(shape) != 4 or shape[1] != 3:
        raise ValueError(f"pixel_values must be [n,3,224,224], got {shape}")
    _check_size(shape[2], shape[3], interpolate_pos_encoding)
    if dtype in (torch.float32, np.dtype("float32")):
        return PIX_F32_NCHW
    if dtype == torch.bfloat16:
        return PIX_BF16_NCHW
    raise TypeError(f"unsupported pixel dtype {dtype} (float32, bfloat16 or uint8)")


def _pixel_hw(t: Union[torch.Tensor, np.ndarray], fmt: int) -> Tuple[int, int]:
    return (int(t.shape[1]), int(t.shape[2])) if fmt == PIX_U8_NHWC else (int(t.shape[2]), int(t.shape[3]))


def vision_seq_len(height: int, width: int) -> int:
    return (height // PATCH) * (width // PATCH) + 1


def _ids_dtype(dtype) -> int:
    if dtype in (torch.int64, np.dtype("int64")):
        return IDS_I64
    if dtype in (torch.int32, np.dtype("int32")):
        return IDS_I32
    raise TypeError(f"input_ids must be int32 or int64, got {dtype}")


def _check_ids(input_ids, attention_mask) -> Tuple[int, int]:
    if len(input_ids.shape) != 2:
        raise ValueError(f"input_ids must be [n, seq_len], got {tuple(input_ids.shape)}")
    n, s = int(input_ids.shape[0]), int(input_ids.shape[1])
    if s > MAX_TEXT_LEN:
        raise ValueError(
            "Sequence length must be less than max_position_embeddings (got `sequence length`: "
            f"{s} and max_position_embeddings: {MAX_TEXT_LEN}")
    if attention_mask is not None and tuple(attention_mask.shape) != (n, s):
        raise ValueError(f"attention_mask shape {tuple(attention_mask.shape)} != input_ids shape {(n, s)}")
    return n, s


WINDOW = IMAGE_SIZE


def check_region(region: Union[torch.Tensor, np.ndarray]) -> Tuple[int, int, int]:
    if region.dtype not in (torch.uint8, np.dtype("uint8")):
        raise ValueError(f"a region must be uint8 RGB [H, W, 3], got dtype {region.dtype}")
    shape = tuple(region.shape)
    if len(shape) != 3 or shape[2] != 3:
        raise ValueError(f"a region must be uint8 RGB [H, W, 3], got shape {shape}")
    h, w = int(shape[0]), int(shape[1])
    if h < WINDOW or w < WINDOW:
        raise ValueError(f"region {h}x{w} is smaller than one {WINDOW}x{WINDOW} window")
    strides = region.stride() if torch.is_tensor(region) else tuple(s // region.itemsize for s in region.strides)
    if strides[2] != 1 or strides[1] != 3 or strides[0] < 3 * w:
        raise ValueError(f"a region needs packed RGB pixels (strides (>= 3 * W, 3, 1) in bytes), got strides {strides}")
    return h, w, int(strides[0])


def check_origins(origins, height: int, width: int) -> np.ndarray:
    o = np.asarray(origins.cpu() if torch.is_tensor(origins) else origins)
    if o.size == 0:
        return np.zeros((0, 2), np.int32)
    if o.ndim != 2 or o.shape[1] != 2 or o.dtype.kind not in "iu":
        raise ValueError(f"origins must be integer [n, 2] (row, col), got {o.dtype} {o.shape}")
    bad = (o[:, 0] < 0) | (o[:, 1] < 0) | (o[:, 0] > height - WINDOW) | (o[:, 1] > width - WINDOW)
    if bad.any():
        i = int(np.flatnonzero(bad)[0])
        raise ValueError(f"window {i} at ({int(o[i, 0])}, {int(o[i, 1])}) is outside the {height}x{width} region "
                         f"(rows 0..{height - WINDOW}, columns 0..{width - WINDOW})")
    return np.ascontiguousarray(o, dtype=np.int32)


def _device_region(region) -> Tuple[int, int, int]:
    if not (torch.is_tensor(region) and region.is_cuda):
        raise ValueError("the region must be a CUDA tensor here; host regions go through plip_b200.regions.encode_region")
    return check_region(region)


@torch.no_grad()
def window_background_counts(region: torch.Tensor, origins, threshold: int = 200) -> torch.Tensor:
    h, w, pitch = _device_region(region)
    o = check_origins(origins, h, w)
    n = int(o.shape[0])
    out = torch.empty(n, device=region.device, dtype=torch.int32)
    if n:
        with torch.cuda.device(region.device):
            check(lib().plip_window_background_counts(region.data_ptr(), h, w, pitch, o.ctypes.data, n, int(threshold),
                                                      out.data_ptr(), torch.cuda.current_stream(region.device).cuda_stream),
                  "plip_window_background_counts")
    return out


def _packed_u8(t, what: str, channels) -> Tuple[int, int, int, int]:
    if t.dtype not in (torch.uint8, np.dtype("uint8")):
        raise ValueError(f"{what} must be uint8, got dtype {t.dtype}")
    shape = tuple(t.shape)
    c = shape[2] if len(shape) == 3 else 1
    if len(shape) not in (2, 3) or c not in channels:
        raise ValueError(f"{what} must be uint8 {' or '.join('[H, W]' if k == 1 else f'[H, W, {k}]' for k in channels)}"
                         f", got shape {shape}")
    h, w = int(shape[0]), int(shape[1])
    if h < 1 or w < 1:
        raise ValueError(f"{what} is empty ({h}x{w})")
    strides = tuple(t.stride()) if torch.is_tensor(t) else tuple(s // t.itemsize for s in t.strides)
    if (len(shape) == 3 and strides[2] != 1) or strides[1] != c or strides[0] < c * w:
        raise ValueError(f"{what} needs packed pixels (strides (>= {c} * W, {c}{', 1' if len(shape) == 3 else ''}) in "
                         f"bytes), got strides {strides}")
    return h, w, c, int(strides[0])


MAX_RESIZE = 65536
_RC_BAD_ARGUMENT = -2


def _check_args(rc: int, what: str) -> None:
    if rc == _RC_BAD_ARGUMENT:
        from ._lib import last_error
        raise ValueError(f"{what}: {last_error()}")
    check(rc, what)


def resize_filter_bounds(in_size: int, out_size: int) -> np.ndarray:
    if not (1 <= in_size <= MAX_RESIZE and 1 <= out_size <= MAX_RESIZE):
        raise ValueError(f"resize sizes {in_size} -> {out_size} are outside 1..{MAX_RESIZE}")
    b = np.zeros((out_size, 2), np.int32)
    check(lib().plip_resize_filter_bounds(int(in_size), int(out_size), b.ctypes.data), "plip_resize_filter_bounds")
    return b


class ResizeWorkspace:

    def __init__(self, device):
        self.device, self.buf = torch.device(device), None

    def get(self, nbytes: int) -> torch.Tensor:
        if self.buf is None or self.buf.numel() < nbytes:
            self.buf = torch.empty(nbytes, dtype=torch.uint8, device=self.device)
        return self.buf


@torch.no_grad()
def resize_rows(band: torch.Tensor, src_row0: int, height: int, new_h: int, new_w: int, rows: Tuple[int, int],
                out: torch.Tensor, workspace: Optional[ResizeWorkspace] = None) -> torch.Tensor:
    if not (torch.is_tensor(band) and band.is_cuda):
        raise ValueError("resize_rows: the source must be a CUDA tensor")
    bh, w, _, pitch = _packed_u8(band, "the source", (3,))
    o0, o1 = int(rows[0]), int(rows[1])
    if not (1 <= height <= MAX_RESIZE and 1 <= w <= MAX_RESIZE and 1 <= new_h <= MAX_RESIZE and 1 <= new_w <= MAX_RESIZE):
        raise ValueError(f"resize {height}x{w} -> {new_h}x{new_w}: sizes must be in 1..{MAX_RESIZE}")
    if not 0 <= o0 < o1 <= new_h:
        raise ValueError(f"output rows [{o0}, {o1}) are not a non-empty range of 0..{new_h}")
    if not (0 <= src_row0 and src_row0 + bh <= height):
        raise ValueError(f"a band of {bh} rows at row {src_row0} is not inside the {height} source rows")
    if not (torch.is_tensor(out) and out.is_cuda and out.device == band.device):
        raise ValueError(f"the output must be a CUDA tensor on {band.device}")
    oh, ow, _, opitch = _packed_u8(out, "the output", (3,))
    if (oh, ow) != (o1 - o0, new_w):
        raise ValueError(f"the output is {oh}x{ow}, rows [{o0}, {o1}) of width {new_w} need {o1 - o0}x{new_w}")
    L = lib()
    need = C.c_uint64(0)
    _check_args(L.plip_resize_region_workspace(int(height), w, int(new_h), int(new_w), o0, o1, C.byref(need)),
                "plip_resize_region_workspace")
    ws = (workspace or ResizeWorkspace(band.device)).get(int(need.value))
    with torch.cuda.device(band.device):
        _check_args(L.plip_resize_region_u8(band.data_ptr(), pitch, int(src_row0), bh, int(height), w, out.data_ptr(),
                                            opitch, int(new_h), int(new_w), o0, o1, ws.data_ptr(), ws.numel(),
                                            torch.cuda.current_stream(band.device).cuda_stream), "plip_resize_region_u8")
    return out


def resize_region(region: torch.Tensor, new_h: int, new_w: int, out: Optional[torch.Tensor] = None) -> torch.Tensor:
    if not (torch.is_tensor(region) and region.is_cuda):
        raise ValueError("resize_region: the region must be a CUDA tensor")
    h = _packed_u8(region, "a region", (3,))[0]
    if out is None:
        if not (1 <= new_h <= MAX_RESIZE and 1 <= new_w <= MAX_RESIZE):
            raise ValueError(f"output size {new_h}x{new_w} is outside 1..{MAX_RESIZE}")
        out = torch.empty((int(new_h), int(new_w), 3), dtype=torch.uint8, device=region.device)
    return resize_rows(region, 0, h, int(new_h), int(new_w), (0, int(new_h)), out)


def _device_tiles(t, what: str) -> int:
    if not (torch.is_tensor(t) and t.is_cuda and t.dtype == torch.uint8 and t.dim() == 4
            and tuple(t.shape[1:]) == (IMAGE_SIZE, IMAGE_SIZE, 3) and t.is_contiguous()):
        raise ValueError(f"{what} must be a contiguous CUDA uint8 [n,224,224,3] tensor, got "
                         f"{getattr(t, 'dtype', type(t))} {tuple(getattr(t, 'shape', ()))}")
    return int(t.shape[0])


@torch.no_grad()
def resize_crop(src: torch.Tensor, descs: np.ndarray, out: Optional[torch.Tensor] = None) -> torch.Tensor:
    from .preprocess import RESIZE_DESC_DTYPE
    assert src.is_cuda and src.dtype == torch.uint8 and src.is_contiguous() and src.dim() == 1
    descs = np.ascontiguousarray(descs, dtype=RESIZE_DESC_DTYPE)
    n = int(descs.shape[0])
    if out is None:
        out = torch.empty((n, 224, 224, 3), device=src.device, dtype=torch.uint8)
    assert out.is_cuda and out.dtype == torch.uint8 and out.is_contiguous() and out.numel() == n * 224 * 224 * 3
    if n:
        with torch.cuda.device(src.device):
            check(lib().plip_resize_crop_u8(src.data_ptr(), int(src.numel()), descs.ctypes.data, n, out.data_ptr(),
                                            torch.cuda.current_stream(src.device).cuda_stream), "plip_resize_crop_u8")
    return out


@torch.no_grad()
def resize_crop_fill(src: torch.Tensor, descs: np.ndarray, out: Optional[torch.Tensor] = None) -> torch.Tensor:
    from .preprocess import RESIZE_DESC_DTYPE
    if not (torch.is_tensor(src) and src.is_cuda and src.dtype == torch.uint8 and src.is_contiguous()
            and src.dim() == 1):
        raise ValueError("resize_crop_fill: src must be a contiguous 1-D CUDA uint8 tensor")
    descs = np.ascontiguousarray(descs, dtype=RESIZE_DESC_DTYPE).reshape(-1)
    n = int(descs.shape[0])
    if out is None:
        out = torch.empty((n, IMAGE_SIZE, IMAGE_SIZE, 3), device=src.device, dtype=torch.uint8)
    elif _device_tiles(out, "out") != n or out.device != src.device:
        raise ValueError(f"resize_crop_fill: out must be [{n},224,224,3] on {src.device}")
    if n:
        with torch.cuda.device(src.device):
            _check_args(lib().plip_resize_crop_fill_u8(src.data_ptr(), int(src.numel()), descs.ctypes.data, n,
                                                       out.data_ptr(), torch.cuda.current_stream(src.device).cuda_stream),
                        "plip_resize_crop_fill_u8")
    return out


@torch.no_grad()
def mask_value_sets(masks: torch.Tensor, out: Optional[torch.Tensor] = None) -> torch.Tensor:
    if not (torch.is_tensor(masks) and masks.is_cuda and masks.dtype == torch.uint8 and masks.dim() == 4
            and masks.is_contiguous()):
        raise ValueError("mask_value_sets: masks must be a contiguous CUDA uint8 [n, h, w, c] tensor")
    n, h, w, c = (int(x) for x in masks.shape)
    if out is None:
        out = torch.empty((n, c, 8), dtype=torch.int32, device=masks.device)
    elif not (out.is_cuda and out.dtype == torch.int32 and tuple(out.shape) == (n, c, 8) and out.is_contiguous()
              and out.device == masks.device):
        raise ValueError(f"mask_value_sets: out must be a contiguous int32 [{n}, {c}, 8] tensor on {masks.device}")
    if n:
        with torch.cuda.device(masks.device):
            _check_args(lib().plip_mask_value_sets_u8(masks.data_ptr(), n, h, w, c, out.data_ptr(),
                                                      torch.cuda.current_stream(masks.device).cuda_stream),
                        "plip_mask_value_sets_u8")
    return out


@torch.no_grad()
def warp_tiles(tiles: torch.Tensor, params: np.ndarray, out: Optional[torch.Tensor] = None) -> torch.Tensor:
    from .preprocess import WARP_DESC_DTYPE
    n = _device_tiles(tiles, "tiles")
    params = np.ascontiguousarray(params, dtype=WARP_DESC_DTYPE).reshape(-1)
    if params.shape[0] != n:
        raise ValueError(f"warp_tiles: {params.shape[0]} descriptors for {n} tiles")
    if out is None:
        out = torch.empty_like(tiles)
    elif _device_tiles(out, "out") != n or out.device != tiles.device:
        raise ValueError(f"warp_tiles: out must be [{n},224,224,3] on {tiles.device}")
    if n:
        with torch.cuda.device(tiles.device):
            _check_args(lib().plip_warp_tiles_u8(tiles.data_ptr(), out.data_ptr(), params.ctypes.data, n,
                                                 torch.cuda.current_stream(tiles.device).cuda_stream),
                        "plip_warp_tiles_u8")
    return out


@torch.no_grad()
def window_mask_counts(mask: torch.Tensor, origins, threshold: int = 10) -> torch.Tensor:
    if not (torch.is_tensor(mask) and mask.is_cuda):
        raise ValueError("window_mask_counts: the mask must be a CUDA tensor")
    h, w, c, pitch = _packed_u8(mask, "a mask", (1, 3))
    if h < WINDOW or w < WINDOW:
        raise ValueError(f"mask {h}x{w} is smaller than one {WINDOW}x{WINDOW} window")
    if not -(2 ** 31) <= int(threshold) < 2 ** 31:
        raise ValueError(f"threshold {threshold} does not fit int32")
    o = check_origins(origins, h, w)
    n = int(o.shape[0])
    out = torch.empty(n, device=mask.device, dtype=torch.int32)
    if n:
        with torch.cuda.device(mask.device):
            check(lib().plip_window_mask_counts(mask.data_ptr(), h, w, c, pitch, o.ctypes.data, n, int(threshold),
                                                out.data_ptr(), torch.cuda.current_stream(mask.device).cuda_stream),
                  "plip_window_mask_counts")
    return out


@torch.no_grad()
def similarity_topk(query: torch.Tensor, space: torch.Tensor, k: int, scale: float = 1.0, normalize_query: bool = True,
                    normalize_space: bool = False, device: Union[int, str, torch.device, None] = None):
    if not torch.cuda.is_available():
        raise RuntimeError("plip_b200 needs a CUDA device (sm_90a); there is no CPU fallback")
    dev = torch.device("cuda", torch.cuda.current_device()) if device is None else torch.device(device)
    L = lib()
    q = query.to(torch.float32).to(dev, non_blocking=True).contiguous()
    s = space.to(torch.float32).to(dev, non_blocking=True).contiguous()
    n = int(q.shape[0])
    idx = torch.empty(n, k, device=dev, dtype=torch.int32)
    val = torch.empty(n, k, device=dev, dtype=torch.float32)
    if n == 0:
        return idx, val
    with torch.cuda.device(dev):
        check(L.plip_similarity_topk(q.data_ptr(), n, s.data_ptr(), int(s.shape[0]), C.c_float(scale), int(normalize_query),
                                     int(normalize_space), int(k), idx.data_ptr(), val.data_ptr(),
                                     torch.cuda.current_stream(dev).cuda_stream), "plip_similarity_topk")
    return idx, val


def sgd_shuffle_permutation(n: int, seed: int) -> np.ndarray:
    if not 1 <= int(n) < 2 ** 31:
        raise ValueError(f"n = {n} is outside 1..2^31-1")
    out = np.empty(int(n), np.int32)
    check(lib().plip_sgd_shuffle_permutation(int(n), int(seed) & 0xFFFFFFFF, out.ctypes.data),
          "plip_sgd_shuffle_permutation")
    return out


def _device_embeddings(x: torch.Tensor, what: str) -> Tuple[int, int]:
    if not (torch.is_tensor(x) and x.is_cuda and x.dtype == torch.float32 and x.dim() == 2 and x.is_contiguous()):
        raise ValueError(f"{what} must be a contiguous CUDA float32 [n, {EMBED_DIM}] tensor")
    return int(x.shape[0]), int(x.shape[1])


@torch.no_grad()
def sgd_fit(x: torch.Tensor, class_ids, n_classes: int, problems, sigma, max_iter: int = 10000, tol: float = 1e-3,
            n_iter_no_change: int = 5):
    n, d = _device_embeddings(x, "x")
    cls = np.ascontiguousarray(np.asarray(class_ids), dtype=np.int32)
    sig = np.ascontiguousarray(np.asarray(sigma), dtype=np.int32)
    if cls.shape != (n,) or sig.ndim != 2 or sig.shape[1] != n:
        raise ValueError(f"class ids {cls.shape} and sigma {sig.shape} do not match n = {n}")
    table = (_SgdProblem * len(problems))(*[_SgdProblem(float(a), float(wp), float(wn), int(pc), int(si))
                                            for a, pc, wp, wn, si in problems])
    p = len(problems)
    L = lib()
    need = C.c_uint64(0)
    _check_args(L.plip_sgd_workspace_bytes(n, int(sig.shape[0]), p, C.byref(need)), "plip_sgd_workspace_bytes")
    dev = x.device
    ws = torch.empty(int(need.value), dtype=torch.uint8, device=dev)
    coef = torch.empty(p, EMBED_DIM, dtype=torch.float32, device=dev)
    intercept = torch.empty(p, dtype=torch.float64, device=dev)
    n_iter = torch.empty(p, dtype=torch.int32, device=dev)
    overflow = torch.empty(p, dtype=torch.int32, device=dev)
    with torch.cuda.device(dev):
        _check_args(L.plip_sgd_fit(x.data_ptr(), n, d, cls.ctypes.data, int(n_classes), table, p, sig.ctypes.data,
                                   int(sig.shape[0]), int(max_iter), C.c_double(tol), int(n_iter_no_change),
                                   coef.data_ptr(), intercept.data_ptr(), n_iter.data_ptr(), overflow.data_ptr(),
                                   ws.data_ptr(), ws.numel(), torch.cuda.current_stream(dev).cuda_stream), "plip_sgd_fit")
    return coef, intercept, n_iter, overflow


@torch.no_grad()
def linear_decision(x: torch.Tensor, coef: torch.Tensor, intercept: torch.Tensor):
    n, d = _device_embeddings(x, "x")
    c, dc = _device_embeddings(coef, "coef")
    b = intercept.to(device=x.device, dtype=torch.float64).contiguous()
    if coef.device != x.device or dc != d or b.shape != (c,):
        raise ValueError(f"coef {tuple(coef.shape)} on {coef.device} and intercept {tuple(intercept.shape)} do not "
                         f"match x on {x.device}")
    scores = torch.empty(n, c, dtype=torch.float32, device=x.device)
    pred = torch.empty(n, dtype=torch.int32, device=x.device)
    with torch.cuda.device(x.device):
        _check_args(lib().plip_linear_decision(x.data_ptr(), n, d, coef.data_ptr(), b.data_ptr(), c, scores.data_ptr(),
                                               pred.data_ptr(), torch.cuda.current_stream(x.device).cuda_stream),
                    "plip_linear_decision")
    return scores, pred


class Engine:

    def __init__(self, state_dict: Mapping[str, torch.Tensor], device: Union[int, str, torch.device, None] = None,
                 max_micro_batch: int = 1024, operand_dtype="bf16"):
        if not torch.cuda.is_available():
            raise RuntimeError("plip_b200 needs a CUDA device (sm_90a); there is no CPU fallback")
        self._L = lib()
        dev = torch.device("cuda", torch.cuda.current_device()) if device is None else torch.device(device)
        if dev.type != "cuda":
            raise RuntimeError(f"plip_b200 runs on CUDA devices only, got {dev}")
        self.device = torch.device("cuda", dev.index if dev.index is not None else torch.cuda.current_device())
        fmt, _ = operand_format(operand_dtype)
        self.operand_dtype = "fp16" if fmt == 1 else "bf16"
        blob, scale = pack_state_dict(state_dict, self.operand_dtype)
        self.logit_scale_exp = float(scale)
        h = C.c_void_p()
        with torch.cuda.device(self.device):
            torch.cuda.init()
            check(self._L.plip_create_ex(blob.data_ptr(), blob.numel(), C.c_float(scale), self.device.index,
                                         int(max_micro_batch), fmt, C.byref(h)), "plip_create_ex")
        self._h = h
        self.max_micro_batch = int(max_micro_batch)

    def set_text_pooling(self, no_eos_argmax: bool) -> None:
        check(self._L.plip_set_text_pooling(self._h, int(bool(no_eos_argmax))), "plip_set_text_pooling")

    def set_last_layer_pruning(self, on: bool) -> None:
        check(self._L.plip_set_last_layer_pruning(self._h, int(bool(on))), "plip_set_last_layer_pruning")

    @property
    def last_layer_pruning(self) -> bool:
        return bool(self._L.plip_last_layer_pruning(self._h))

    def close(self) -> None:
        if getattr(self, "_h", None):
            self._L.plip_destroy(self._h)
            self._h = None

    def __del__(self):
        try:
            self.close()
        except Exception:
            pass

    def _stream(self) -> int:
        return torch.cuda.current_stream(self.device).cuda_stream

    def _dev(self, t: torch.Tensor) -> torch.Tensor:
        if t.device != self.device:
            t = t.to(self.device, non_blocking=True)
        return t.contiguous()

    def upload_async(self, t: torch.Tensor):
        if getattr(self, "_copy_stream", None) is None:
            self._copy_stream = torch.cuda.Stream(device=self.device)
        cur = torch.cuda.current_stream(self.device)
        with torch.cuda.stream(self._copy_stream):
            d = t.contiguous().to(self.device, non_blocking=True)
            ev = torch.cuda.Event()
            ev.record(self._copy_stream)
        d.record_stream(cur)
        return d, ev

    @torch.no_grad()
    def encode_images(self, pixels: torch.Tensor, normalize: bool = False,
                      interpolate_pos_encoding: bool = False) -> torch.Tensor:
        fmt = _pixel_format(pixels, interpolate_pos_encoding)
        n = int(pixels.shape[0])
        if n == 0:
            return torch.empty(0, EMBED_DIM, device=self.device)
        pixels = self._dev(pixels)
        out = torch.empty(n, EMBED_DIM, device=self.device, dtype=torch.float32)
        h, w = _pixel_hw(pixels, fmt)
        with torch.cuda.device(self.device):
            check(self._L.plip_encode_images_hw(self._h, pixels.data_ptr(), fmt, n, h, w, out.data_ptr(),
                                                int(normalize), self._stream()), "plip_encode_images_hw")
        return out

    @torch.no_grad()
    def encode_windows(self, region: torch.Tensor, origins, normalize: bool = False) -> torch.Tensor:
        h, w, pitch = _device_region(region)
        o = check_origins(origins, h, w)
        n = int(o.shape[0])
        out = torch.empty(n, EMBED_DIM, device=self.device, dtype=torch.float32)
        if n:
            if region.device != self.device:
                raise ValueError(f"the region is on {region.device}, the engine on {self.device}")
            with torch.cuda.device(self.device):
                check(self._L.plip_encode_windows(self._h, region.data_ptr(), h, w, pitch, o.ctypes.data, n,
                                                  out.data_ptr(), int(normalize), self._stream()), "plip_encode_windows")
        return out

    def window_background_counts(self, region: torch.Tensor, origins, threshold: int = 200) -> torch.Tensor:
        return window_background_counts(region, origins, threshold)

    @torch.no_grad()
    def encode_text(self, input_ids: torch.Tensor, attention_mask: Optional[torch.Tensor] = None,
                    normalize: bool = False, prefix_len: Optional[int] = None) -> torch.Tensor:
        n, s = _check_ids(input_ids, attention_mask)
        p_len = s if prefix_len is None else int(prefix_len)
        if not 1 <= p_len <= s:
            raise ValueError(f"prefix_len {p_len} out of [1, {s}]")
        if n == 0:
            return torch.empty(0, EMBED_DIM, device=self.device)
        idt = _ids_dtype(input_ids.dtype)
        ids = self._dev(input_ids)
        mask = None
        if attention_mask is not None:
            mask = self._dev(attention_mask.to(input_ids.dtype))
        out = torch.empty(n, EMBED_DIM, device=self.device, dtype=torch.float32)
        with torch.cuda.device(self.device):
            check(self._L.plip_encode_text_prefix(self._h, ids.data_ptr(), idt,
                                                  mask.data_ptr() if mask is not None else None, n, s, p_len,
                                                  out.data_ptr(), int(normalize), self._stream()), "plip_encode_text")
        return out

    @torch.no_grad()
    def similarity(self, image_embeds: torch.Tensor, text_embeds: torch.Tensor, scale: Optional[float] = None,
                   normalize_image: bool = True, normalize_text: bool = True) -> torch.Tensor:
        a = self._dev(image_embeds.to(torch.float32))
        b = self._dev(text_embeds.to(torch.float32))
        if a.shape[-1] != EMBED_DIM or b.shape[-1] != EMBED_DIM:
            raise ValueError("embeddings must have 512 columns")
        n, m = int(a.shape[0]), int(b.shape[0])
        ld = (m + 127) // 128 * 128
        out = torch.empty(n, ld, device=self.device, dtype=torch.float32)
        if n == 0 or m == 0:
            return out[:, :m]
        s = self.logit_scale_exp if scale is None else float(scale)
        with torch.cuda.device(self.device):
            check(self._L.plip_similarity(a.data_ptr(), n, b.data_ptr(), m, C.c_float(s), int(normalize_image),
                                          int(normalize_text), out.data_ptr(), ld, self._stream()), "plip_similarity")
        return out[:, :m]

    @torch.no_grad()
    def similarity_topk(self, query: torch.Tensor, space: torch.Tensor, k: int, scale: float = 1.0,
                        normalize_query: bool = True, normalize_space: bool = False):
        return similarity_topk(query, space, k, scale, normalize_query, normalize_space, device=self.device)

    @torch.no_grad()
    def l2_normalize_(self, x: torch.Tensor) -> torch.Tensor:
        assert x.is_cuda and x.dtype == torch.float32 and x.is_contiguous()
        if x.shape[0]:
            with torch.cuda.device(self.device):
                check(self._L.plip_l2_normalize(x.data_ptr(), int(x.shape[0]), int(x.shape[1]), self._stream()),
                      "plip_l2_normalize")
        return x

    @torch.no_grad()
    def resize_crop(self, src: torch.Tensor, descs: np.ndarray, out: Optional[torch.Tensor] = None) -> torch.Tensor:
        return resize_crop(src, descs, out)

    def _outputs(self, n: int, S: int, D: int, heads: int, output_hidden_states: bool, output_attentions: bool,
                 last_hidden_from_hidden: bool):
        from ._lib import TowerOutputs
        f32 = dict(device=self.device, dtype=torch.float32)
        out = {"embeds": torch.empty(n, EMBED_DIM, **f32), "pooler_output": torch.empty(n, D, **f32),
               "hidden": torch.empty(NUM_LAYERS + 1, n, S, D, **f32) if output_hidden_states else None,
               "attn": torch.empty(NUM_LAYERS, n, heads, S, S, **f32) if output_attentions else None}
        if last_hidden_from_hidden and out["hidden"] is not None:
            out["last_hidden_state"] = out["hidden"][NUM_LAYERS]
        else:
            out["last_hidden_state"] = torch.empty(n, S, D, **f32)
        own_last = out["hidden"] is None or not last_hidden_from_hidden
        ptr = lambda t: t.data_ptr() if t is not None else None
        st = TowerOutputs(ptr(out["embeds"]), ptr(out["pooler_output"]),
                          ptr(out["last_hidden_state"]) if own_last else None, ptr(out["hidden"]), ptr(out["attn"]), 0)
        return st, out

    @staticmethod
    def _outputs_result(out) -> Dict[str, object]:
        hid, att = out.pop("hidden"), out.pop("attn")
        out["hidden_states"] = tuple(hid.unbind(0)) if hid is not None else None
        out["attentions"] = tuple(att.unbind(0)) if att is not None else None
        return out

    @torch.no_grad()
    def vision_outputs(self, pixels: torch.Tensor, output_hidden_states: bool = False, output_attentions: bool = False,
                       interpolate_pos_encoding: bool = False, normalize: bool = False) -> Dict[str, object]:
        fmt = _pixel_format(pixels, interpolate_pos_encoding)
        h, w = _pixel_hw(pixels, fmt)
        n, S = int(pixels.shape[0]), vision_seq_len(h, w)
        st, out = self._outputs(n, S, VISION_DIM, VISION_HEADS, output_hidden_states, output_attentions, True)
        st.normalize = int(bool(normalize))
        if n:
            pixels = self._dev(pixels)
            with torch.cuda.device(self.device):
                check(self._L.plip_vision_outputs(self._h, pixels.data_ptr(), fmt, n, h, w, C.byref(st),
                                                  self._stream()), "plip_vision_outputs")
        return self._outputs_result(out)

    @torch.no_grad()
    def text_outputs(self, input_ids: torch.Tensor, attention_mask: Optional[torch.Tensor] = None,
                     output_hidden_states: bool = False, output_attentions: bool = False,
                     normalize: bool = False) -> Dict[str, object]:
        n, s = _check_ids(input_ids, attention_mask)
        idt = _ids_dtype(input_ids.dtype)
        st, out = self._outputs(n, s, TEXT_DIM, TEXT_HEADS, output_hidden_states, output_attentions, False)
        st.normalize = int(bool(normalize))
        if n:
            ids = self._dev(input_ids)
            mask = self._dev(attention_mask.to(input_ids.dtype)) if attention_mask is not None else None
            with torch.cuda.device(self.device):
                check(self._L.plip_text_outputs(self._h, ids.data_ptr(), idt,
                                                mask.data_ptr() if mask is not None else None, n, s, C.byref(st),
                                                self._stream()), "plip_text_outputs")
        return self._outputs_result(out)

    def encode_images_host(self, pixels: Union[np.ndarray, torch.Tensor], normalize: bool = False,
                           out: Optional[torch.Tensor] = None) -> torch.Tensor:
        fmt = _pixel_format(pixels)
        t = torch.from_numpy(np.ascontiguousarray(pixels)) if isinstance(pixels, np.ndarray) else pixels.contiguous()
        assert not t.is_cuda, "encode_images_host takes host memory; use encode_images for device tensors"
        n = int(t.shape[0])
        if out is None:
            out = torch.empty(n, EMBED_DIM, dtype=torch.float32)
        if n:
            check(self._L.plip_encode_images_host(self._h, t.data_ptr(), fmt, n, out.data_ptr(), int(normalize)),
                  "plip_encode_images_host")
        return out

    def encode_text_host(self, input_ids: Union[np.ndarray, torch.Tensor], attention_mask=None,
                         normalize: bool = False, out: Optional[torch.Tensor] = None) -> torch.Tensor:
        ids = torch.from_numpy(np.ascontiguousarray(input_ids)) if isinstance(input_ids, np.ndarray) else input_ids.contiguous()
        n, s = _check_ids(ids, attention_mask)
        idt = _ids_dtype(ids.dtype)
        mask = None
        if attention_mask is not None:
            mask = (torch.from_numpy(np.ascontiguousarray(attention_mask)) if isinstance(attention_mask, np.ndarray)
                    else attention_mask).to(ids.dtype).contiguous()
        if out is None:
            out = torch.empty(n, EMBED_DIM, dtype=torch.float32)
        if n:
            check(self._L.plip_encode_text_host(self._h, ids.data_ptr(), idt, mask.data_ptr() if mask is not None else None,
                                                n, s, out.data_ptr(), int(normalize)), "plip_encode_text_host")
        return out

    def profile(self, on: bool) -> None:
        check(self._L.plip_profile_enable(self._h, int(bool(on))), "plip_profile_enable")

    def profile_read(self):
        from ._lib import KernelTime
        buf = (KernelTime * 64)()
        cnt = C.c_int(0)
        check(self._L.plip_profile_read(self._h, buf, 64, C.byref(cnt)), "plip_profile_read")
        return [{"name": buf[i].name.decode(), "launches": int(buf[i].launches), "total_ms": float(buf[i].total_ms),
                 "flops": float(buf[i].flops), "bytes": float(buf[i].bytes)} for i in range(min(cnt.value, 64))]

    @torch.no_grad()
    def hidden_states(self, tower: str, inputs: torch.Tensor, num_layers: int,
                      attention_mask: Optional[torch.Tensor] = None,
                      interpolate_pos_encoding: bool = False) -> torch.Tensor:
        x = self._dev(inputs)
        n = int(x.shape[0])
        if tower == "vision":
            fmt = _pixel_format(x, interpolate_pos_encoding)
            h, w = _pixel_hw(x, fmt)
            out = torch.empty((n, vision_seq_len(h, w), 768), device=self.device, dtype=torch.float32)
            with torch.cuda.device(self.device):
                check(self._L.plip_dbg_hidden_states_hw(self._h, x.data_ptr(), fmt, n, h, w, int(num_layers),
                                                        out.data_ptr(), self._stream()), "plip_dbg_hidden_states_hw")
            return out
        assert x.shape[1] == 77
        mask = self._dev(attention_mask.to(x.dtype)) if attention_mask is not None else None
        out = torch.empty((n, 77, 512), device=self.device, dtype=torch.float32)
        with torch.cuda.device(self.device):
            check(self._L.plip_dbg_hidden_states(self._h, 1, x.data_ptr(), _ids_dtype(x.dtype),
                                                 mask.data_ptr() if mask is not None else None, n, int(num_layers),
                                                 out.data_ptr(), self._stream()), "plip_dbg_hidden_states")
        return out
```

### plip_b200/modeling.py

```python
from __future__ import annotations

from dataclasses import dataclass
from typing import Mapping, Optional, Tuple, Union

import torch

from .engine import Engine


@dataclass
class BaseModelOutputWithPooling:

    last_hidden_state: torch.Tensor
    pooler_output: torch.Tensor
    hidden_states: Optional[Tuple[torch.Tensor, ...]] = None
    attentions: Optional[Tuple[torch.Tensor, ...]] = None

    def __getitem__(self, k):
        return getattr(self, k)

    def keys(self):
        return tuple(k for k in ("last_hidden_state", "pooler_output", "hidden_states", "attentions")
                     if getattr(self, k) is not None)


@dataclass
class CLIPOutput:

    logits_per_image: torch.Tensor
    logits_per_text: torch.Tensor
    text_embeds: torch.Tensor
    image_embeds: torch.Tensor
    loss: Optional[torch.Tensor] = None
    text_model_output: Optional[BaseModelOutputWithPooling] = None
    vision_model_output: Optional[BaseModelOutputWithPooling] = None

    def __getitem__(self, k):
        return getattr(self, k)

    def keys(self):
        return ("logits_per_image", "logits_per_text", "text_embeds", "image_embeds") + tuple(
            k for k in ("text_model_output", "vision_model_output") if getattr(self, k) is not None)


def _model_output(o) -> BaseModelOutputWithPooling:
    return BaseModelOutputWithPooling(last_hidden_state=o["last_hidden_state"], pooler_output=o["pooler_output"],
                                      hidden_states=o["hidden_states"], attentions=o["attentions"])


class PlipCLIPModel:

    def __init__(self, state_dict: Mapping[str, torch.Tensor], device: Union[int, str, torch.device, None] = None,
                 max_micro_batch: int = 1024, operand_dtype="bf16"):
        self.engine = Engine(state_dict, device=device, max_micro_batch=max_micro_batch, operand_dtype=operand_dtype)
        self.device = self.engine.device
        self.training = False

    @classmethod
    def from_pretrained(cls, name_or_path: str, device=None, max_micro_batch: int = 1024, operand_dtype="bf16",
                        **hf_kwargs):
        from transformers import CLIPModel

        tok = hf_kwargs.pop("use_auth_token", None)
        if tok is not None:
            hf_kwargs.setdefault("token", tok)
        hf = CLIPModel.from_pretrained(name_or_path, **hf_kwargs)
        cfg = hf.config
        v, t = cfg.vision_config, cfg.text_config
        want = {"vision hidden_size": (v.hidden_size, 768), "vision patch_size": (v.patch_size, 32),
                "vision image_size": (v.image_size, 224), "vision num_hidden_layers": (v.num_hidden_layers, 12),
                "vision num_attention_heads": (v.num_attention_heads, 12), "vision intermediate_size": (v.intermediate_size, 3072),
                "vision hidden_act": (v.hidden_act, "quick_gelu"), "vision layer_norm_eps": (float(v.layer_norm_eps), 1e-5),
                "text hidden_size": (t.hidden_size, 512), "text num_hidden_layers": (t.num_hidden_layers, 12),
                "text num_attention_heads": (t.num_attention_heads, 8), "text intermediate_size": (t.intermediate_size, 2048),
                "text hidden_act": (t.hidden_act, "quick_gelu"), "text layer_norm_eps": (float(t.layer_norm_eps), 1e-5),
                "text max_position_embeddings": (t.max_position_embeddings, 77), "text vocab_size": (t.vocab_size, 49408),
                "projection_dim": (cfg.projection_dim, 512)}
        bad = {k: got for k, (got, exp) in want.items() if got != exp}
        if bad:
            raise ValueError("plip_b200 implements the CLIP ViT-B/32 geometry only (PLIP's architecture); this "
                             f"checkpoint differs in {bad}")
        m = cls(hf.state_dict(), device=device, max_micro_batch=max_micro_batch, operand_dtype=operand_dtype)
        m.engine.set_text_pooling(getattr(t, "eos_token_id", 49407) == 2)
        return m

    @classmethod
    def from_openai_state_dict(cls, state_dict, device=None, max_micro_batch: int = 1024, operand_dtype="bf16"):
        m = cls(state_dict, device=device, max_micro_batch=max_micro_batch, operand_dtype=operand_dtype)
        m.engine.set_text_pooling(True)
        return m

    def to(self, *args, **kwargs):
        return self

    def eval(self):
        return self

    def float(self):
        return self

    @property
    def logit_scale_exp(self) -> float:
        return self.engine.logit_scale_exp

    def get_image_features(self, pixel_values: torch.Tensor = None, interpolate_pos_encoding: bool = False,
                           **_ignored) -> torch.Tensor:
        if pixel_values is None:
            raise ValueError("You have to specify pixel_values")
        return self.engine.encode_images(pixel_values, interpolate_pos_encoding=interpolate_pos_encoding)

    def get_text_features(self, input_ids: torch.Tensor = None, attention_mask: Optional[torch.Tensor] = None,
                          **_ignored) -> torch.Tensor:
        if input_ids is None:
            raise ValueError("You have to specify input_ids")
        return self.engine.encode_text(input_ids, attention_mask)

    def vision_model(self, pixel_values: torch.Tensor = None, output_hidden_states: bool = False,
                     output_attentions: bool = False, interpolate_pos_encoding: bool = False) -> BaseModelOutputWithPooling:
        if pixel_values is None:
            raise ValueError("You have to specify pixel_values")
        return _model_output(self.engine.vision_outputs(pixel_values, bool(output_hidden_states), bool(output_attentions),
                                                        interpolate_pos_encoding))

    def text_model(self, input_ids: torch.Tensor = None, attention_mask: Optional[torch.Tensor] = None,
                   output_hidden_states: bool = False, output_attentions: bool = False) -> BaseModelOutputWithPooling:
        if input_ids is None:
            raise ValueError("You have to specify input_ids")
        return _model_output(self.engine.text_outputs(input_ids, attention_mask, bool(output_hidden_states),
                                                      bool(output_attentions)))

    def forward(self, input_ids: torch.Tensor = None, pixel_values: torch.Tensor = None,
                attention_mask: Optional[torch.Tensor] = None, return_loss: Optional[bool] = None,
                interpolate_pos_encoding: bool = False, output_hidden_states: Optional[bool] = None,
                output_attentions: Optional[bool] = None, **_ignored) -> CLIPOutput:
        if input_ids is None:
            raise ValueError("You have to specify input_ids")
        if pixel_values is None:
            raise ValueError("You have to specify pixel_values")
        ipe = interpolate_pos_encoding
        vout = tout = None
        if output_hidden_states or output_attentions:
            ohs, oa = bool(output_hidden_states), bool(output_attentions)
            vo = self.engine.vision_outputs(pixel_values, ohs, oa, ipe, normalize=True)
            to = self.engine.text_outputs(input_ids, attention_mask, ohs, oa, normalize=True)
            img, txt = vo.pop("embeds"), to.pop("embeds")
            vout, tout = _model_output(vo), _model_output(to)
        elif not pixel_values.is_cuda:
            mb = self.engine.max_micro_batch
            parts = [self.engine.upload_async(pixel_values[i:i + mb]) for i in range(0, pixel_values.shape[0], mb)]
            txt = self.engine.encode_text(input_ids, attention_mask, normalize=True)
            embs = []
            for chunk, uploaded in parts:
                torch.cuda.current_stream(self.device).wait_event(uploaded)
                embs.append(self.engine.encode_images(chunk, normalize=True, interpolate_pos_encoding=ipe))
            img = embs[0] if len(embs) == 1 else torch.cat(embs, dim=0)
        else:
            img = self.engine.encode_images(pixel_values, normalize=True, interpolate_pos_encoding=ipe)
            txt = self.engine.encode_text(input_ids, attention_mask, normalize=True)
        lpi = self.engine.similarity(img, txt, normalize_image=False, normalize_text=False)
        loss = None
        if return_loss:
            lpt = lpi.t()
            tgt = torch.arange(lpt.shape[0], device=lpt.device)
            loss = (torch.nn.functional.cross_entropy(lpt, tgt) + torch.nn.functional.cross_entropy(lpt.t(), tgt)) / 2
        return CLIPOutput(logits_per_image=lpi, logits_per_text=lpi.t(), text_embeds=txt, image_embeds=img, loss=loss,
                          text_model_output=tout, vision_model_output=vout)

    __call__ = forward

    def encode_image(self, images: torch.Tensor) -> torch.Tensor:
        return self.engine.encode_images(images)

    def encode_text(self, idx: torch.Tensor) -> torch.Tensor:
        return self.engine.encode_text(idx)
```

Before: 26310.

## Encode image and text towers concurrently on forked streams with separate workspaces

Adds plip_encode_pair, which runs the vision and text towers of a CLIP forward concurrently: the text tower gets its own workspace and a non-blocking side stream joined to the main stream with fork/join events. Layer code is refactored into per-stage functions parameterized by a Tower/Workspace struct so the two towers no longer share scratch buffers. The goal is to fill idle SMs while the smaller text tower runs, instead of serializing it after vision. It costs an extra workspace allocation, and it falls back to sequential encoding when a batch exceeds the micro-batch limit or is eligible for the graph path.

```diff
diff --git a/include/plip_b200.h b/include/plip_b200.h
--- a/include/plip_b200.h
+++ b/include/plip_b200.h
@@ -82,6 +82,10 @@
 PLIP_API int plip_encode_text_prefix(plip_engine_t* e, const void* ids_dev, int ids_dtype,
                                      const void* attention_mask_dev, int64_t n, int seq_len, int prefix_len,
                                      float* out_dev, int normalize, void* stream);
+
+PLIP_API int plip_encode_pair(plip_engine_t* e, const void* pixels_dev, int pixel_format, int64_t n_img,
+                              const void* ids_dev, int ids_dtype, const void* attention_mask_dev, int64_t n_txt,
+                              int seq_len, float* img_out_dev, float* txt_out_dev, int normalize, void* stream);
 
 typedef struct plip_tower_outputs {
   float* embeds;
diff --git a/plip_b200/_lib.py b/plip_b200/_lib.py
--- a/plip_b200/_lib.py
+++ b/plip_b200/_lib.py
@@ -88,6 +88,7 @@
     "plip_window_background_counts": (_i, [_vp, _i, _i, _i64, _vp, _i64, _i, _vp, _vp]),
     "plip_encode_text": (_i, [_vp, _vp, _i, _vp, _i64, _i, _fp, _i, _vp]),
     "plip_encode_text_prefix": (_i, [_vp, _vp, _i, _vp, _i64, _i, _i, _fp, _i, _vp]),
+    "plip_encode_pair": (_i, [_vp, _vp, _i, _i64, _vp, _i, _vp, _i64, _i, _fp, _fp, _i, _vp]),
     "plip_vision_outputs": (_i, [_vp, _vp, _i, _i64, _i, _i, C.POINTER(TowerOutputs), _vp]),
     "plip_text_outputs": (_i, [_vp, _vp, _i, _vp, _i64, _i, C.POINTER(TowerOutputs), _vp]),
     "plip_similarity": (_i, [_fp, _i64, _fp, _i64, _f, _i, _i, _fp, _i64, _vp]),
diff --git a/plip_b200/csrc/engine.cu b/plip_b200/csrc/engine.cu
--- a/plip_b200/csrc/engine.cu
+++ b/plip_b200/csrc/engine.cu
@@ -135,6 +135,18 @@
   bool operator<(const GraphKey& o) const { return fields() < o.fields(); }
 };
 
+struct Workspace {
+  float* X = nullptr;
+  __nv_bfloat16* Xn = nullptr;
+  __nv_bfloat16* AO = nullptr;
+  float2* stats = nullptr;
+  __nv_bfloat16* QKV = nullptr;
+  __nv_bfloat16* H = nullptr;
+  __nv_bfloat16* pooled = nullptr;
+  int32_t* row_idx = nullptr;
+  int32_t* kmask = nullptr;
+};
+
 struct Graph {
   cudaGraphExec_t exec = nullptr;
   unsigned long long kernels = 0;
@@ -159,15 +171,9 @@
   LayerW vis[kLayers], txt[kLayers];
   const float *t_tok = nullptr, *t_pos = nullptr, *t_fin_g = nullptr, *t_fin_b = nullptr;
   const __nv_bfloat16* t_proj = nullptr;
-  float* X = nullptr;
-  __nv_bfloat16* Xn = nullptr;
-  __nv_bfloat16* AO = nullptr;
-  float2* stats = nullptr;
-  __nv_bfloat16* QKV = nullptr;
-  __nv_bfloat16* H = nullptr;
-  __nv_bfloat16* pooled = nullptr;
-  int32_t* row_idx = nullptr;
-  int32_t* kmask = nullptr;
+  Workspace ws, ws_txt;
+  cudaStream_t s_txt = nullptr;
+  cudaEvent_t ev_fork = nullptr, ev_join = nullptr;
   cudaEvent_t ev_last = nullptr;
   cudaStream_t s_compute = nullptr, s_copy = nullptr;
   cudaEvent_t ev_copied[2] = {nullptr, nullptr}, ev_done[2] = {nullptr, nullptr};
@@ -253,8 +259,8 @@
   size_t x, xn, ao, stats, qkv, h, pooled, rowidx, kmask, total;
 };
 
-WsLayout ws_layout(int mb) {
-  const size_t rv = (size_t)mb * kVisSeq, rt = (size_t)mb * kTxtSeq;
+WsLayout ws_layout(int mb, bool vision = true) {
+  const size_t rv = vision ? (size_t)mb * kVisSeq : 0, rt = (size_t)mb * kTxtSeq;
   auto mx = [](size_t a, size_t b) { return a > b ? a : b; };
   auto al = [](size_t a) { return (a + 1023) & ~(size_t)1023; };
   WsLayout w;
@@ -264,12 +270,26 @@
   w.ao = off; off += al(mx(rv * kVisDim, rt * kTxtDim) * 2);
   w.stats = off; off += al(mx(rv, rt) * kStatSlots * sizeof(float2));
   w.qkv = off; off += al(mx(rv * 3 * kVisDim, rt * 3 * kTxtDim) * 2);
-  w.h = off; off += al(mx(mx(rv * kVisFF, rt * kTxtFF), (size_t)mb * kPatches * kPatchK) * 2);
+  w.h = off; off += al(mx(mx(rv * kVisFF, rt * kTxtFF), vision ? (size_t)mb * kPatches * kPatchK : 0) * 2);
   w.pooled = off; off += al((size_t)mb * kVisDim * 2);
   w.rowidx = off; off += al((size_t)mb * 4);
   w.kmask = off; off += al(rt * 4);
   w.total = off;
   return w;
+}
+
+Workspace bind_workspace(uint8_t* base, const WsLayout& w) {
+  Workspace ws;
+  ws.X = reinterpret_cast<float*>(base + w.x);
+  ws.Xn = reinterpret_cast<__nv_bfloat16*>(base + w.xn);
+  ws.AO = reinterpret_cast<__nv_bfloat16*>(base + w.ao);
+  ws.stats = reinterpret_cast<float2*>(base + w.stats);
+  ws.QKV = reinterpret_cast<__nv_bfloat16*>(base + w.qkv);
+  ws.H = reinterpret_cast<__nv_bfloat16*>(base + w.h);
+  ws.pooled = reinterpret_cast<__nv_bfloat16*>(base + w.pooled);
+  ws.row_idx = reinterpret_cast<int32_t*>(base + w.rowidx);
+  ws.kmask = reinterpret_cast<int32_t*>(base + w.kmask);
+  return ws;
 }
 
 int gemm(plip_engine* e, int kind, GemmArgs g, cudaStream_t st) {
@@ -280,22 +300,93 @@
   return launch_gemm(g, st);
 }
 
-int layer_tail(plip_engine* e, const LayerW& w, int rows, int D, int FF, const __nv_bfloat16* ao, float* x, bool last,
-               int& np, cudaStream_t st) {
+struct Tower {
+  int id;
+  const LayerW* L;
+  Workspace w;
+  int64_t n_seq;
+  int S, D, FF, heads;
+  bool causal;
+  const int32_t* kmask;
+  int np;
+  int64_t rows() const { return n_seq * S; }
+};
+
+Tower vision_tower(const plip_engine* e, const Workspace& w, int64_t mb, int S) {
+  return Tower{0, e->vis, w, mb, S, kVisDim, kVisFF, kVisHeads, false, nullptr, 1};
+}
+
+Tower text_tower(const plip_engine* e, const Workspace& w, int64_t mb, int S, const int32_t* kmask) {
+  return Tower{1, e->txt, w, mb, S, kTxtDim, kTxtFF, kTxtHeads, true, kmask, 1};
+}
+
+int stage_rowstats(plip_engine* e, Tower& t, cudaStream_t st) {
+  e->prof_tower = t.id;
+  const int64_t M = t.rows();
+  ProfScope ps(e, st, PK_ROWSTATS, 0, (double)M * t.D * 6 + (double)M * 8);
+  t.np = 1;
+  return launch_rowstats_cast(t.w.X, M, t.D, t.w.Xn, t.w.stats, e->f16, st);
+}
+
+GemmArgs qkv_args(const Tower& t, int l) {
+  const LayerW& w = t.L[l];
   GemmArgs g;
-  g.A = ao; g.lda = D; g.W = w.wo; g.ldw = D; g.M = rows; g.N = D; g.K = D;
-  g.bias = w.bo; g.out = x; g.ldo = D; g.epi = EPI_BIAS_RESID_F32;
-  g.xb_out = e->Xn; g.stats_out = e->stats; g.n_tiles_used = &np;
-  if (int rc = gemm(e, PK_OUT, g, st)) return rc;
-  g = GemmArgs();
-  g.A = e->Xn; g.lda = D; g.W = w.w1; g.ldw = D; g.M = rows; g.N = FF; g.K = D;
-  g.bias = w.b1; g.colsum = w.s1; g.stats_in = e->stats; g.n_partials = np;
-  g.out = e->H; g.ldo = FF; g.epi = EPI_LN_BIAS_GELU_BF16;
-  if (int rc = gemm(e, PK_FC1, g, st)) return rc;
-  g = GemmArgs();
-  g.A = e->H; g.lda = FF; g.W = w.w2; g.ldw = FF; g.M = rows; g.N = D; g.K = FF;
-  g.bias = w.b2; g.out = x; g.ldo = D; g.epi = EPI_BIAS_RESID_F32;
-  if (!last) { g.xb_out = e->Xn; g.stats_out = e->stats; g.n_tiles_used = &np; }
+  g.A = t.w.Xn; g.lda = t.D; g.W = w.wqkv; g.ldw = t.D; g.M = (int)t.rows(); g.N = 3 * t.D; g.K = t.D;
+  g.bias = w.bqkv; g.colsum = w.sqkv; g.stats_in = t.w.stats; g.n_partials = t.np;
+  g.out = t.w.QKV; g.ldo = 3 * t.D; g.epi = EPI_LN_BIAS_BF16;
+  return g;
+}
+
+GemmArgs out_args(Tower& t, int l) {
+  const LayerW& w = t.L[l];
+  GemmArgs g;
+  g.A = t.w.AO; g.lda = t.D; g.W = w.wo; g.ldw = t.D; g.M = (int)t.rows(); g.N = t.D; g.K = t.D;
+  g.bias = w.bo; g.out = t.w.X; g.ldo = t.D; g.epi = EPI_BIAS_RESID_F32;
+  g.xb_out = t.w.Xn; g.stats_out = t.w.stats; g.n_tiles_used = &t.np;
+  return g;
+}
+
+int stage_qkv(plip_engine* e, Tower& t, int l, cudaStream_t st) {
+  e->prof_tower = t.id;
+  return gemm(e, PK_QKV, qkv_args(t, l), st);
+}
+
+int stage_attn(plip_engine* e, Tower& t, int l, float* attn, cudaStream_t st) {
+  e->prof_tower = t.id;
+  const int64_t M = t.rows();
+  const double b_att = (double)M * 3 * t.D * 2 + (double)M * t.D * 2;
+  const double f_att = 4.0 * (double)t.n_seq * t.heads * t.S * t.S * kHeadDim;
+  {
+    ProfScope ps(e, st, t.S > 128 ? PK_ATTN_LONG : PK_ATTN, f_att, b_att);
+    if (int rc = launch_attention(t.w.QKV, t.n_seq, t.S, t.heads, t.causal, t.kmask, t.w.AO, e->f16, st)) return rc;
+  }
+  if (!attn) return 0;
+  ProfScope ps(e, st, PK_ATTN_PROBS, 0.5 * f_att, (double)M * 2 * t.D * 2 + (double)t.n_seq * t.heads * t.S * t.S * 4);
+  return launch_attention_probs(t.w.QKV, t.n_seq, t.S, t.heads, t.causal, t.kmask, attn, e->f16, st);
+}
+
+int stage_out(plip_engine* e, Tower& t, int l, cudaStream_t st) {
+  e->prof_tower = t.id;
+  return gemm(e, PK_OUT, out_args(t, l), st);
+}
+
+int stage_fc1(plip_engine* e, Tower& t, int l, cudaStream_t st) {
+  e->prof_tower = t.id;
+  const LayerW& w = t.L[l];
+  GemmArgs g;
+  g.A = t.w.Xn; g.lda = t.D; g.W = w.w1; g.ldw = t.D; g.M = (int)t.rows(); g.N = t.FF; g.K = t.D;
+  g.bias = w.b1; g.colsum = w.s1; g.stats_in = t.w.stats; g.n_partials = t.np;
+  g.out = t.w.H; g.ldo = t.FF; g.epi = EPI_LN_BIAS_GELU_BF16;
+  return gemm(e, PK_FC1, g, st);
+}
+
+int stage_fc2(plip_engine* e, Tower& t, int l, bool last, cudaStream_t st) {
+  e->prof_tower = t.id;
+  const LayerW& w = t.L[l];
+  GemmArgs g;
+  g.A = t.w.H; g.lda = t.FF; g.W = w.w2; g.ldw = t.FF; g.M = (int)t.rows(); g.N = t.D; g.K = t.FF;
+  g.bias = w.b2; g.out = t.w.X; g.ldo = t.D; g.epi = EPI_BIAS_RESID_F32;
+  if (!last) { g.xb_out = t.w.Xn; g.stats_out = t.w.stats; g.n_tiles_used = &t.np; }
   return gemm(e, PK_FC2, g, st);
 }
 
@@ -327,108 +418,98 @@
   return p;
 }
 
-int run_layers(plip_engine* e, const LayerW* L, int64_t n_seq, int S, int D, int FF, int heads, bool causal,
-               const int32_t* kmask, int num_layers, cudaStream_t st, bool prune = false,
+int run_layers(plip_engine* e, Tower& t, int num_layers, cudaStream_t st, bool prune = false,
                const int32_t* pool_idx = nullptr, const PassOut& out = PassOut(), const float** pooled_x = nullptr) {
-  const int64_t M = n_seq * S;
+  const int64_t M = t.rows();
   PLIP_REQUIRE(M <= 0x7fffffff / 4, "micro-batch too large");
   PLIP_REQUIRE(!prune || (pooled_x && !out.hidden && !out.attn), "internal: per-layer outputs of a pruned pass");
-  const size_t x_bytes = (size_t)M * D * 4;
-  if (out.hidden) PLIP_CUDA_CHECK(cudaMemcpyAsync(out.hidden, e->X, x_bytes, cudaMemcpyDeviceToDevice, st));
+  const size_t x_bytes = (size_t)M * t.D * 4;
+  if (out.hidden) PLIP_CUDA_CHECK(cudaMemcpyAsync(out.hidden, t.w.X, x_bytes, cudaMemcpyDeviceToDevice, st));
   if (num_layers <= 0) return 0;
-  {
-    ProfScope ps(e, st, PK_ROWSTATS, 0, (double)M * D * 6 + (double)M * 8);
-    if (int rc = launch_rowstats_cast(e->X, M, D, e->Xn, e->stats, e->f16, st)) return rc;
-  }
-  const double b_att = (double)M * 3 * D * 2 + (double)M * D * 2;
-  const double f_att = 4.0 * (double)n_seq * heads * S * S * kHeadDim;
-  int np = 1;
+  if (int rc = stage_rowstats(e, t, st)) return rc;
   for (int l = 0; l < num_layers; ++l) {
-    const LayerW& w = L[l];
     const bool last = l + 1 == num_layers;
-    GemmArgs g;
-    g.A = e->Xn; g.lda = D; g.W = w.wqkv; g.ldw = D; g.M = (int)M; g.N = 3 * D; g.K = D;
-    g.bias = w.bqkv; g.colsum = w.sqkv; g.stats_in = e->stats; g.n_partials = np;
-    g.out = e->QKV; g.ldo = 3 * D; g.epi = EPI_LN_BIAS_BF16;
-    if (int rc = gemm(e, PK_QKV, g, st)) return rc;
-    {
-      ProfScope ps(e, st, S > 128 ? PK_ATTN_LONG : PK_ATTN, f_att, b_att);
-      if (int rc = launch_attention(e->QKV, n_seq, S, heads, causal, kmask, e->AO, e->f16, st)) return rc;
-    }
-    if (out.attn) {
-      ProfScope ps(e, st, PK_ATTN_PROBS, 0.5 * f_att, (double)M * 2 * D * 2 + (double)n_seq * heads * S * S * 4);
-      if (int rc = launch_attention_probs(e->QKV, n_seq, S, heads, causal, kmask, out.attn + l * out.attn_stride,
-                                          e->f16, st)) return rc;
-    }
+    if (int rc = stage_qkv(e, t, l, st)) return rc;
+    if (int rc = stage_attn(e, t, l, out.attn ? out.attn + l * out.attn_stride : nullptr, st)) return rc;
     if (!(prune && last)) {
-      if (int rc = layer_tail(e, w, (int)M, D, FF, e->AO, e->X, last, np, st)) return rc;
+      if (int rc = stage_out(e, t, l, st)) return rc;
+      if (int rc = stage_fc1(e, t, l, st)) return rc;
+      if (int rc = stage_fc2(e, t, l, last, st)) return rc;
       if (out.hidden)
-        PLIP_CUDA_CHECK(cudaMemcpyAsync(out.hidden + (l + 1) * out.hidden_stride, e->X, x_bytes,
+        PLIP_CUDA_CHECK(cudaMemcpyAsync(out.hidden + (l + 1) * out.hidden_stride, t.w.X, x_bytes,
                                         cudaMemcpyDeviceToDevice, st));
       continue;
     }
-    __nv_bfloat16* ao_p = e->QKV;
-    float* x_p = reinterpret_cast<float*>(reinterpret_cast<uint8_t*>(e->QKV) + (((size_t)n_seq * D * 2 + 1023) & ~(size_t)1023));
+    Tower c = t;
+    c.S = 1;
+    c.w.AO = t.w.QKV;
+    c.w.X = reinterpret_cast<float*>(reinterpret_cast<uint8_t*>(t.w.QKV) +
+                                     (((size_t)t.n_seq * t.D * 2 + 1023) & ~(size_t)1023));
     {
-      ProfScope ps(e, st, PK_MISC, 0, (double)n_seq * D * 12);
-      if (int rc = launch_gather_rows(e->AO, e->X, pool_idx, S, n_seq, D, ao_p, x_p, st)) return rc;
+      ProfScope ps(e, st, PK_MISC, 0, (double)t.n_seq * t.D * 12);
+      if (int rc = launch_gather_rows(t.w.AO, t.w.X, pool_idx, t.S, t.n_seq, t.D, c.w.AO, c.w.X, st)) return rc;
     }
-    if (int rc = layer_tail(e, w, (int)n_seq, D, FF, ao_p, x_p, true, np, st)) return rc;
-    *pooled_x = x_p;
-  }
-  return 0;
-}
-
-int vision_trunk(plip_engine* e, const VisInput& in, int64_t mb, const VisGeom& geo, int num_layers,
-                 cudaStream_t st, bool prune = false, const PassOut& out = PassOut(),
-                 const float** pooled_x = nullptr) {
+    if (int rc = stage_out(e, c, l, st)) return rc;
+    if (int rc = stage_fc1(e, c, l, st)) return rc;
+    if (int rc = stage_fc2(e, c, l, true, st)) return rc;
+    *pooled_x = c.w.X;
+  }
+  return 0;
+}
+
+int vision_embed(plip_engine* e, const VisInput& in, int64_t mb, const VisGeom& geo, cudaStream_t st) {
   e->prof_tower = 0;
+  const Workspace& w = e->ws;
   const double dmb = (double)mb;
   const int patches = geo.gh * geo.gw;
   const float* pos = e->v_pos;
   if (geo.gh != kGrid || geo.gw != kGrid) {
-    float* table = reinterpret_cast<float*>(e->QKV);
+    float* table = reinterpret_cast<float*>(w.QKV);
     ProfScope ps(e, st, PK_MISC, 0, (double)kVisSeq * kVisDim * 4 + (double)geo.S * kVisDim * 4);
     if (int rc = launch_pos_interp(e->v_pos, geo.gh, geo.gw, table, st)) return rc;
     pos = table;
   }
   {
     ProfScope ps(e, st, PK_IM2COL, 0, dmb * (double)pixel_bytes(in.fmt, geo.H, geo.W) + dmb * patches * kPatchK * 2);
-    const int rc = in.win.region ? launch_window_im2col(in.win, mb, e->H, e->f16, st)
-                                 : launch_im2col(in.pixels, in.fmt, mb, geo.H, geo.W, e->H, e->f16, st);
+    const int rc = in.win.region ? launch_window_im2col(in.win, mb, w.H, e->f16, st)
+                                 : launch_im2col(in.pixels, in.fmt, mb, geo.H, geo.W, w.H, e->f16, st);
     if (rc) return rc;
   }
   GemmArgs g;
-  g.A = e->H; g.lda = kPatchK; g.W = e->v_patch_w; g.ldw = kPatchK;
+  g.A = w.H; g.lda = kPatchK; g.W = e->v_patch_w; g.ldw = kPatchK;
   g.M = (int)(mb * patches); g.N = kVisDim; g.K = kPatchK;
-  g.out = e->X; g.ldo = kVisDim; g.pos = pos; g.patches = patches; g.seq = geo.S; g.epi = EPI_PATCH_F32;
+  g.out = w.X; g.ldo = kVisDim; g.pos = pos; g.patches = patches; g.seq = geo.S; g.epi = EPI_PATCH_F32;
   if (int rc = gemm(e, PK_PATCH, g, st)) return rc;
   {
     ProfScope ps(e, st, PK_MISC, 0, dmb * kVisDim * 4);
-    if (int rc = launch_cls_rows(e->v_cls, pos, mb, geo.S, e->X, st)) return rc;
+    if (int rc = launch_cls_rows(e->v_cls, pos, mb, geo.S, w.X, st)) return rc;
   }
   const int64_t M = mb * geo.S;
-  {
-    ProfScope ps(e, st, PK_LN, 0, (double)M * kVisDim * 8);
-    if (int rc = launch_layernorm(e->X, nullptr, kVisDim, M, kVisDim, e->v_pre_g, e->v_pre_b, e->X, nullptr, e->f16, st)) return rc;
-  }
-  return run_layers(e, e->vis, mb, geo.S, kVisDim, kVisFF, kVisHeads, false, nullptr, num_layers, st, prune, nullptr,
-                    out, pooled_x);
-}
-
-int pooled_head(plip_engine* e, const float* pooled_x, const int32_t* pool_idx, int64_t mb, int S, int D,
-                const float* gamma, const float* beta, const __nv_bfloat16* proj, float* out, int normalize,
+  ProfScope ps(e, st, PK_LN, 0, (double)M * kVisDim * 8);
+  return launch_layernorm(w.X, nullptr, kVisDim, M, kVisDim, e->v_pre_g, e->v_pre_b, w.X, nullptr, e->f16, st);
+}
+
+int vision_trunk(plip_engine* e, const VisInput& in, int64_t mb, const VisGeom& geo, int num_layers,
+                 cudaStream_t st, bool prune = false, const PassOut& out = PassOut(),
+                 const float** pooled_x = nullptr) {
+  if (int rc = vision_embed(e, in, mb, geo, st)) return rc;
+  Tower t = vision_tower(e, e->ws, mb, geo.S);
+  return run_layers(e, t, num_layers, st, prune, nullptr, out, pooled_x);
+}
+
+int pooled_head(plip_engine* e, const Workspace& w, const float* pooled_x, const int32_t* pool_idx, int64_t mb, int S,
+                int D, const float* gamma, const float* beta, const __nv_bfloat16* proj, float* out, int normalize,
                 cudaStream_t st, float* pooled_f32) {
   {
     ProfScope ps(e, st, PK_LN, 0, (double)mb * D * (pooled_f32 ? 10 : 6));
     const bool compact = pooled_x != nullptr;
-    if (int rc = launch_layernorm(compact ? pooled_x : e->X, compact ? nullptr : pool_idx,
+    if (int rc = launch_layernorm(compact ? pooled_x : w.X, compact ? nullptr : pool_idx,
                                   compact || pool_idx ? (int64_t)D : (int64_t)S * D, mb, D, gamma, beta, pooled_f32,
-                                  e->pooled, e->f16, st)) return rc;
+                                  w.pooled, e->f16, st)) return rc;
   }
   if (!out) return 0;
   GemmArgs g;
-  g.A = e->pooled; g.lda = D; g.W = proj; g.ldw = D;
+  g.A = w.pooled; g.lda = D; g.W = proj; g.ldw = D;
   g.M = (int)mb; g.N = kProj; g.K = D; g.out = out; g.ldo = kProj; g.epi = EPI_F32;
   if (int rc = gemm(e, PK_PROJ, g, st)) return rc;
   if (normalize) {
@@ -438,48 +519,85 @@
   return 0;
 }
 
+int vision_head(plip_engine* e, const float* pooled_x, int64_t mb, int S, const PassOut& out, cudaStream_t st) {
+  e->prof_tower = 0;
+  return pooled_head(e, e->ws, pooled_x, nullptr, mb, S, kVisDim, e->v_post_g, e->v_post_b, e->v_proj, out.embeds,
+                     out.normalize, st, out.pooled);
+}
+
 int vision_pass(plip_engine* e, const VisInput& in, int64_t mb, const VisGeom& geo, const PassOut& out, bool prune,
                 cudaStream_t st) {
   const float* pooled_x = nullptr;
   if (int rc = vision_trunk(e, in, mb, geo, kLayers, st, prune, out, &pooled_x)) return rc;
   if (out.last_hidden)
-    PLIP_CUDA_CHECK(cudaMemcpyAsync(out.last_hidden, e->X, (size_t)mb * geo.S * kVisDim * 4, cudaMemcpyDeviceToDevice,
-                                    st));
+    PLIP_CUDA_CHECK(cudaMemcpyAsync(out.last_hidden, e->ws.X, (size_t)mb * geo.S * kVisDim * 4,
+                                    cudaMemcpyDeviceToDevice, st));
   if (!out.embeds && !out.pooled) return 0;
-  return pooled_head(e, pooled_x, nullptr, mb, geo.S, kVisDim, e->v_post_g, e->v_post_b, e->v_proj, out.embeds,
-                     out.normalize, st, out.pooled);
-}
-
-int text_trunk(plip_engine* e, const void* ids, int ids_dtype, const void* mask, int64_t mb, int S, int stride,
-               int num_layers, cudaStream_t st, bool prune = false, const PassOut& out = PassOut(),
-               const float** pooled_x = nullptr) {
+  return vision_head(e, pooled_x, mb, geo.S, out, st);
+}
+
+int text_embed(plip_engine* e, const Workspace& w, const void* ids, int ids_dtype, const void* mask, int64_t mb, int S,
+               int stride, cudaStream_t st, Tower* t) {
   e->prof_tower = 1;
   {
     ProfScope ps(e, st, PK_EMBED, 0, (double)mb * S * kTxtDim * 8);
-    if (int rc = launch_text_embed(ids, ids_dtype, mb, S, stride, e->t_tok, e->t_pos, e->X, e->row_idx, kEosId, e->text_pool_argmax, st)) return rc;
+    if (int rc = launch_text_embed(ids, ids_dtype, mb, S, stride, e->t_tok, e->t_pos, w.X, w.row_idx, kEosId,
+                                   e->text_pool_argmax, st)) return rc;
   }
   const int32_t* km = nullptr;
   if (mask) {
     ProfScope ps(e, st, PK_MISC, 0, (double)mb * S * 12);
-    if (int rc = launch_mask_to_i32(mask, ids_dtype, mb * S, S, stride, e->kmask, st)) return rc;
-    km = e->kmask;
-  }
-  return run_layers(e, e->txt, mb, S, kTxtDim, kTxtFF, kTxtHeads, true, km, num_layers, st, prune, e->row_idx, out,
-                    pooled_x);
-}
-
-int text_pass(plip_engine* e, const void* ids, int ids_dtype, const void* mask, int64_t mb, int S, int stride,
-              const PassOut& out, bool prune, cudaStream_t st) {
+    if (int rc = launch_mask_to_i32(mask, ids_dtype, mb * S, S, stride, w.kmask, st)) return rc;
+    km = w.kmask;
+  }
+  *t = text_tower(e, w, mb, S, km);
+  return 0;
+}
+
+int text_trunk(plip_engine* e, const Workspace& w, const void* ids, int ids_dtype, const void* mask, int64_t mb,
+               int S, int stride, int num_layers, cudaStream_t st, bool prune = false, const PassOut& out = PassOut(),
+               const float** pooled_x = nullptr) {
+  Tower t;
+  if (int rc = text_embed(e, w, ids, ids_dtype, mask, mb, S, stride, st, &t)) return rc;
+  return run_layers(e, t, num_layers, st, prune, w.row_idx, out, pooled_x);
+}
+
+int text_head(plip_engine* e, const Workspace& w, const float* pooled_x, int64_t mb, int S, const PassOut& out,
+              cudaStream_t st) {
+  e->prof_tower = 1;
+  return pooled_head(e, w, pooled_x, w.row_idx, mb, S, kTxtDim, e->t_fin_g, e->t_fin_b, e->t_proj, out.embeds,
+                     out.normalize, st, out.pooled);
+}
+
+int text_pass(plip_engine* e, const Workspace& w, const void* ids, int ids_dtype, const void* mask, int64_t mb, int S,
+              int stride, const PassOut& out, bool prune, cudaStream_t st) {
   const float* pooled_x = nullptr;
-  if (int rc = text_trunk(e, ids, ids_dtype, mask, mb, S, stride, kLayers, st, prune, out, &pooled_x)) return rc;
+  if (int rc = text_trunk(e, w, ids, ids_dtype, mask, mb, S, stride, kLayers, st, prune, out, &pooled_x)) return rc;
   if (out.last_hidden) {
     ProfScope ps(e, st, PK_LN, 0, (double)mb * S * kTxtDim * 8);
-    if (int rc = launch_layernorm(e->X, nullptr, kTxtDim, mb * S, kTxtDim, e->t_fin_g, e->t_fin_b, out.last_hidden,
+    if (int rc = launch_layernorm(w.X, nullptr, kTxtDim, mb * S, kTxtDim, e->t_fin_g, e->t_fin_b, out.last_hidden,
                                   nullptr, e->f16, st)) return rc;
   }
   if (!out.embeds && !out.pooled) return 0;
-  return pooled_head(e, pooled_x, e->row_idx, mb, S, kTxtDim, e->t_fin_g, e->t_fin_b, e->t_proj, out.embeds,
-                     out.normalize, st, out.pooled);
+  return text_head(e, w, pooled_x, mb, S, out, st);
+}
+
+int pair_pass(plip_engine* e, const void* pixels, int fmt, int64_t mb_img, const void* ids, int ids_dtype,
+              const void* mask, int64_t mb_txt, int seq_len, float* out_img, float* out_txt, int normalize, bool prune,
+              cudaStream_t st) {
+  cudaStream_t s_txt = st;
+  if (!e->prof_on) {
+    s_txt = e->s_txt;
+    PLIP_CUDA_CHECK(cudaEventRecord(e->ev_fork, st));
+    PLIP_CUDA_CHECK(cudaStreamWaitEvent(s_txt, e->ev_fork, 0));
+  }
+  if (int rc = text_pass(e, e->ws_txt, ids, ids_dtype, mask, mb_txt, seq_len, seq_len, embeds_only(out_txt, normalize),
+                         prune, s_txt)) return rc;
+  if (s_txt != st) PLIP_CUDA_CHECK(cudaEventRecord(e->ev_join, s_txt));
+  if (int rc = vision_pass(e, tiles(pixels, fmt), mb_img, VisGeom(), embeds_only(out_img, normalize), prune, st))
+    return rc;
+  if (s_txt != st) PLIP_CUDA_CHECK(cudaStreamWaitEvent(st, e->ev_join, 0));
+  return 0;
 }
 
 int ensure_host_path(plip_engine* e) {
@@ -730,8 +848,8 @@
                (long long)per_pass);
   return micro_batches(e, n, n, st, [&](int64_t, int64_t) {
     if (int rc = tower == 0 ? vision_trunk(e, tiles(in, fmt), n, geo, num_layers, st)
-                            : text_trunk(e, in, fmt, mask, n, kTxtSeq, kTxtSeq, num_layers, st)) return rc;
-    PLIP_CUDA_CHECK(cudaMemcpyAsync(hidden, e->X, (size_t)n * S * D * 4, cudaMemcpyDeviceToDevice, st));
+                            : text_trunk(e, e->ws, in, fmt, mask, n, kTxtSeq, kTxtSeq, num_layers, st)) return rc;
+    PLIP_CUDA_CHECK(cudaMemcpyAsync(hidden, e->ws.X, (size_t)n * S * D * 4, cudaMemcpyDeviceToDevice, st));
     return 0;
   });
 }
@@ -799,7 +917,7 @@
   cudaError_t ce = cudaEventCreateWithFlags(&e->ev_last, cudaEventDisableTiming);
   if (ce == cudaSuccess) ce = cudaMalloc(&e->d_blob, nbytes);
   if (ce == cudaSuccess) ce = cudaMalloc(&ws, w.total);
-  e->X = reinterpret_cast<float*>(ws);
+  e->ws.X = reinterpret_cast<float*>(ws);
   if (ce != cudaSuccess) {
     set_last_error("plip_create: allocating %llu (weights) + %llu (workspace) bytes on device %d failed: %s",
                    (unsigned long long)nbytes, (unsigned long long)w.total, device, cudaGetErrorString(ce));
@@ -807,14 +925,7 @@
     plip_destroy(e);
     return -1;
   }
-  e->Xn = reinterpret_cast<__nv_bfloat16*>(ws + w.xn);
-  e->AO = reinterpret_cast<__nv_bfloat16*>(ws + w.ao);
-  e->stats = reinterpret_cast<float2*>(ws + w.stats);
-  e->QKV = reinterpret_cast<__nv_bfloat16*>(ws + w.qkv);
-  e->H = reinterpret_cast<__nv_bfloat16*>(ws + w.h);
-  e->pooled = reinterpret_cast<__nv_bfloat16*>(ws + w.pooled);
-  e->row_idx = reinterpret_cast<int32_t*>(ws + w.rowidx);
-  e->kmask = reinterpret_cast<int32_t*>(ws + w.kmask);
+  e->ws = bind_workspace(ws, w);
   ce = cudaMemcpy(e->d_blob, host_blob, nbytes, cudaMemcpyHostToDevice);
   if (ce != cudaSuccess) {
     set_last_error("plip_create: weight upload failed: %s", cudaGetErrorString(ce));
@@ -834,7 +945,11 @@
   cudaSetDevice(e->device);
   cudaDeviceSynchronize();
   if (e->d_blob) cudaFree(e->d_blob);
-  if (e->X) cudaFree(e->X);
+  if (e->ws.X) cudaFree(e->ws.X);
+  if (e->ws_txt.X) cudaFree(e->ws_txt.X);
+  if (e->s_txt) cudaStreamDestroy(e->s_txt);
+  if (e->ev_fork) cudaEventDestroy(e->ev_fork);
+  if (e->ev_join) cudaEventDestroy(e->ev_join);
   for (int i = 0; i < 2; ++i) {
     if (e->d_in[i]) cudaFree(e->d_in[i]);
     if (e->h_stage[i]) cudaFreeHost(e->h_stage[i]);
@@ -993,14 +1108,49 @@
                        e->text_pool_argmax, e->prune_last};
     return graph_call(e, key, {{{ids_dev, n * row}, {attention_mask_dev, n * row}}}, out_dev, st,
                       [&](cudaStream_t s, const void* ids, const void* mask, float* out) {
-                        return text_pass(e, ids, ids_dtype, mask, n, prefix_len, seq_len, embeds_only(out, normalize),
+                        return text_pass(e, e->ws, ids, ids_dtype, mask, n, prefix_len, seq_len, embeds_only(out, normalize),
                                          prune, s);
                       });
   }
   return micro_batches(e, n, e->max_mb, st, [&](int64_t i, int64_t mb) {
     const uint8_t* mask = attention_mask_dev ? static_cast<const uint8_t*>(attention_mask_dev) + i * row : nullptr;
-    return text_pass(e, static_cast<const uint8_t*>(ids_dev) + i * row, ids_dtype, mask, mb, prefix_len, seq_len,
+    return text_pass(e, e->ws, static_cast<const uint8_t*>(ids_dev) + i * row, ids_dtype, mask, mb, prefix_len, seq_len,
                      embeds_only(out_dev + i * kProj, normalize), prune, st);
+  });
+}
+
+PLIP_API int plip_encode_pair(plip_engine_t* e, const void* pixels_dev, int pixel_format, int64_t n_img,
+                              const void* ids_dev, int ids_dtype, const void* attention_mask_dev, int64_t n_txt,
+                              int seq_len, float* img_out_dev, float* txt_out_dev, int normalize, void* stream) {
+  if (int rc = check_pixels("plip_encode_pair", e, pixels_dev, img_out_dev, pixel_format, n_img, kImage, kImage))
+    return rc;
+  if (int rc = check_ids("plip_encode_pair", e, ids_dev, txt_out_dev, ids_dtype, n_txt, seq_len, seq_len)) return rc;
+  if (n_img > e->max_mb || n_txt > e->max_mb || graph_eligible(e, n_img) || graph_eligible(e, n_txt)) {
+    if (int rc = plip_encode_text(e, ids_dev, ids_dtype, attention_mask_dev, n_txt, seq_len, txt_out_dev, normalize,
+                                  stream)) return rc;
+    return plip_encode_images(e, pixels_dev, pixel_format, n_img, img_out_dev, normalize, stream);
+  }
+  cudaStream_t st = static_cast<cudaStream_t>(stream);
+  if (!e->ws_txt.X) {
+    const WsLayout w = ws_layout(e->max_mb, false);
+    uint8_t* base = nullptr;
+    const cudaError_t ce = cudaMalloc(&base, w.total);
+    if (ce != cudaSuccess) {
+      cudaGetLastError();
+      set_last_error("plip_encode_pair: allocating the %llu-byte text workspace failed: %s",
+                     (unsigned long long)w.total, cudaGetErrorString(ce));
+      return -1;
+    }
+    e->ws_txt = bind_workspace(base, w);
+  }
+  if (!e->s_txt) {
+    PLIP_CUDA_CHECK(cudaStreamCreateWithFlags(&e->s_txt, cudaStreamNonBlocking));
+    PLIP_CUDA_CHECK(cudaEventCreateWithFlags(&e->ev_fork, cudaEventDisableTiming));
+    PLIP_CUDA_CHECK(cudaEventCreateWithFlags(&e->ev_join, cudaEventDisableTiming));
+  }
+  return micro_batches(e, 1, 1, st, [&](int64_t, int64_t) {
+    return pair_pass(e, pixels_dev, pixel_format, n_img, ids_dev, ids_dtype, attention_mask_dev, n_txt, seq_len,
+                     img_out_dev, txt_out_dev, normalize, e->prune_last != 0, st);
   });
 }
 
@@ -1025,7 +1175,7 @@
   cudaStream_t st = static_cast<cudaStream_t>(stream);
   return micro_batches(e, n, e->max_mb, st, [&](int64_t i, int64_t mb) {
     const uint8_t* mask = attention_mask_dev ? static_cast<const uint8_t*>(attention_mask_dev) + i * row : nullptr;
-    return text_pass(e, static_cast<const uint8_t*>(ids_dev) + i * row, ids_dtype, mask, mb, seq_len, seq_len,
+    return text_pass(e, e->ws, static_cast<const uint8_t*>(ids_dev) + i * row, ids_dtype, mask, mb, seq_len, seq_len,
                      pass_out(*outputs, n, i, seq_len, kTxtDim, kTxtHeads), false, st);
   });
 }
diff --git a/plip_b200/distributed.py b/plip_b200/distributed.py
--- a/plip_b200/distributed.py
+++ b/plip_b200/distributed.py
@@ -69,9 +69,10 @@
 class ShardedCLIP:
 
     def __init__(self, encode_images: Callable, encode_text: Callable, similarity: Callable, logit_scale_exp: float,
-                 topk: Optional[Callable] = None):
+                 topk: Optional[Callable] = None, encode_pair: Optional[Callable] = None):
         self.encode_images = encode_images
         self.encode_text = encode_text
+        self.encode_pair = encode_pair
         self.similarity = similarity
         self.topk = topk
         self.logit_scale_exp = float(logit_scale_exp)
@@ -84,9 +85,14 @@
                    lambda a, b, s: engine.similarity(a, b, scale=s, normalize_image=False, normalize_text=False),
                    engine.logit_scale_exp,
                    topk=lambda q, sp, k: engine.similarity_topk(q, sp, k, scale=1.0, normalize_query=False,
-                                                                normalize_space=False))
+                                                                normalize_space=False),
+                   encode_pair=lambda x, ids: engine.encode_pair(x, ids, normalize=True))
 
     def clip_forward(self, local_pixels, local_ids):
+        if self.world_size == 1 and self.encode_pair is not None and torch.is_tensor(local_pixels) \
+                and torch.is_tensor(local_ids):
+            img, txt = self.encode_pair(local_pixels, local_ids)
+            return self.similarity(img, txt, self.logit_scale_exp)
         txt = self.encode_text(local_ids)
         txt_all, work = all_gather_rows_async(txt)
         img = _encode_chunks(self.encode_images, local_pixels)
diff --git a/plip_b200/engine.py b/plip_b200/engine.py
--- a/plip_b200/engine.py
+++ b/plip_b200/engine.py
@@ -521,6 +521,27 @@
         return out
 
     @torch.no_grad()
+    def encode_pair(self, pixels: torch.Tensor, input_ids: torch.Tensor,
+                    attention_mask: Optional[torch.Tensor] = None, normalize: bool = True):
+        fmt = _pixel_format(pixels)
+        n_img = int(pixels.shape[0])
+        n_txt, s = _check_ids(input_ids, attention_mask)
+        if n_img == 0 or n_txt == 0:
+            return (self.encode_images(pixels, normalize=normalize),
+                    self.encode_text(input_ids, attention_mask, normalize=normalize))
+        pixels = self._dev(pixels)
+        ids = self._dev(input_ids)
+        mask = None if attention_mask is None else self._dev(attention_mask.to(input_ids.dtype))
+        img = torch.empty(n_img, EMBED_DIM, device=self.device, dtype=torch.float32)
+        txt = torch.empty(n_txt, EMBED_DIM, device=self.device, dtype=torch.float32)
+        with torch.cuda.device(self.device):
+            check(self._L.plip_encode_pair(self._h, pixels.data_ptr(), fmt, n_img, ids.data_ptr(),
+                                           _ids_dtype(input_ids.dtype), mask.data_ptr() if mask is not None else None,
+                                           n_txt, s, img.data_ptr(), txt.data_ptr(), int(normalize), self._stream()),
+                  "plip_encode_pair")
+        return img, txt
+
+    @torch.no_grad()
     def similarity(self, image_embeds: torch.Tensor, text_embeds: torch.Tensor, scale: Optional[float] = None,
                    normalize_image: bool = True, normalize_text: bool = True) -> torch.Tensor:
         a = self._dev(image_embeds.to(torch.float32))
diff --git a/plip_b200/modeling.py b/plip_b200/modeling.py
--- a/plip_b200/modeling.py
+++ b/plip_b200/modeling.py
@@ -154,6 +154,8 @@
                 torch.cuda.current_stream(self.device).wait_event(uploaded)
                 embs.append(self.engine.encode_images(chunk, normalize=True, interpolate_pos_encoding=ipe))
             img = embs[0] if len(embs) == 1 else torch.cat(embs, dim=0)
+        elif not ipe:
+            img, txt = self.engine.encode_pair(pixel_values, input_ids, attention_mask, normalize=True)
         else:
             img = self.engine.encode_images(pixel_values, normalize=True, interpolate_pos_encoding=ipe)
             txt = self.engine.encode_text(input_ids, attention_mask, normalize=True)
```

After: 27440, median of 6. 4.3% higher.
